# OAID/Tengine

Hardware: AMD Instinct MI355X
Metric: images/sec int8 MobileNet-v1 224x224 (higher is better)
Workload: dtype int8; 1 GPU; mobilenet_v1 int8 batch=1 per GPU (BASELINE configs[1]), weights = seeded synthetic tmfile, input resident in HBM, direct AQL dispatch of the launch list (14 packets per step), 1 stream(s); streams=1, halves=0, global_batch=1, parallelism=dp1, collectives=none

## Files before the change

include/tengine_amd.h:

```cpp
#ifndef TENGINE_AMD_H
#define TENGINE_AMD_H

#include <stddef.h>
#include <stdint.h>

#ifdef __cplusplus
extern "C" {
#endif

#define TAMD_API __attribute__((visibility("default")))

enum { TAMD_DT_FP32 = 0, TAMD_DT_FP16 = 1, TAMD_DT_INT8 = 2, TAMD_DT_UINT8 = 3, TAMD_DT_INT32 = 4 };
enum { TAMD_TT_VAR = 1, TAMD_TT_CONST = 2, TAMD_TT_INPUT = 3 };

enum {
    TAMD_OP_INPUT = 0,
    TAMD_OP_CONST = 1,
    TAMD_OP_CONV = 2,
    TAMD_OP_FC = 3,
    TAMD_OP_POOL = 4,
    TAMD_OP_RELU = 5,
    TAMD_OP_ELTWISE = 6,
    TAMD_OP_CONCAT = 7,
    TAMD_OP_DROPOUT = 8,
    TAMD_OP_UPSAMPLE = 9,
    TAMD_OP_RELU6 = 10,
    TAMD_OP_FLATTEN = 11,
    TAMD_OP_SOFTMAX = 12,
    TAMD_OP_PERMUTE = 13,
    TAMD_OP_RESHAPE = 14,
    TAMD_OP_PRIORBOX = 15,
    TAMD_OP_SIGMOID = 16,
    TAMD_OP_CLIP = 17,
    TAMD_OP_HARDSWISH = 18,
    TAMD_OP_MISH = 19,
    TAMD_OP_INTERP = 20,
    TAMD_OP_SPLIT = 22,
    TAMD_OP_SHUFFLECHANNEL = 23,
    TAMD_OP_PRELU = 25,
    TAMD_OP_SLICE = 26,
    TAMD_OP_NUM
};

typedef struct tamd_conv_param {
    int kernel_h, kernel_w, stride_h, stride_w;
    int pad_h0, pad_h1, pad_w0, pad_w1;
    int dilation_h, dilation_w;
    int input_channel, output_channel, group, activation;
} tamd_conv_param;

typedef struct tamd_fc_param { int num_output; } tamd_fc_param;

typedef struct tamd_pool_param {
    int pool_method, kernel_h, kernel_w, stride_h, stride_w;
    int pad_h0, pad_h1, pad_w0, pad_w1;
    int global, caffe_flavor;
} tamd_pool_param;

typedef struct tamd_relu_param { float negative_slope; } tamd_relu_param;
typedef struct tamd_eltwise_param { int type; int caffe_flavor; float shift, power, scale; } tamd_eltwise_param;
typedef struct tamd_concat_param { int axis; } tamd_concat_param;
typedef struct tamd_upsample_param { float scale; } tamd_upsample_param;
typedef struct tamd_permute_param { int order[4]; } tamd_permute_param;
typedef struct tamd_softmax_param { int axis; } tamd_softmax_param;
typedef struct tamd_reshape_param { int dim_num; int dims[8]; } tamd_reshape_param;
typedef struct tamd_clip_param { float max, min; } tamd_clip_param;
typedef struct tamd_hardswish_param { float alpha, beta; } tamd_hardswish_param;
typedef struct tamd_interp_param { int resize_type; float width_scale, height_scale; int output_width, output_height; } tamd_interp_param;
#define TAMD_SPLIT_MAX 8
typedef struct tamd_split_param { int axis; int num; int sizes[TAMD_SPLIT_MAX]; } tamd_split_param;
typedef struct tamd_shufflechannel_param { int group; } tamd_shufflechannel_param;
typedef struct tamd_slice_param {
    int axis, begin, end, step;
    int iscaffe, ismxnet, isonnx;
    int slice_point_num, begin_num, size_num;
} tamd_slice_param;

#define TAMD_PRIORBOX_MAX 8
typedef struct tamd_priorbox_param {
    int min_size_num, max_size_num, aspect_ratio_num;
    float min_size[TAMD_PRIORBOX_MAX], max_size[TAMD_PRIORBOX_MAX], aspect_ratio[TAMD_PRIORBOX_MAX], variance[4];
    int flip, clip, image_h, image_w;
    float step_h, step_w, offset;
} tamd_priorbox_param;

typedef struct tamd_tensor_desc {
    int dtype;
    int ttype;
    int dim_num;
    int dims[8];
    const void* data;
    int quant_num;
    const float* scales;
    const int* zero_points;
    const char* name;
} tamd_tensor_desc;

typedef struct tamd_node_desc {
    int op;
    int input_num;
    const int* inputs;
    int output_num;
    const int* outputs;
    const void* param;
    const char* name;
} tamd_node_desc;

typedef struct tamd_options {
    const char* dev_name;
    int size;
    int gpu_index;
    int use_hip_graph;
    int profile;
    int direct_dispatch;
    int keep_tensors;
    int u8_integer;
    int split_batch;
} tamd_options;
#define TAMD_OPTIONS_HAS(size, field) ((size) >= (int)(offsetof(tamd_options, field) + sizeof(((const tamd_options*)0)->field)))

typedef struct tamd_graph tamd_graph;

TAMD_API int tamd_device_count(void);
TAMD_API int tamd_init(int gpu_index);
TAMD_API int tamd_shutdown(void);
TAMD_API const char* tamd_last_error(void);
TAMD_API const char* tamd_version(void);
TAMD_API int tamd_op_supported(int op, int dtype);
TAMD_API int tamd_node_supported(const tamd_node_desc* node, const tamd_tensor_desc* inputs, int input_num,
                                 const tamd_tensor_desc* outputs, int output_num);
TAMD_API int tamd_lut_table(int op, int dtype, const void* param, float in_scale, int in_zp, float out_scale, int out_zp,
                            unsigned char table[256]);
TAMD_API int tamd_interp_table(int dtype, float in_scale, int in_zp, float out_scale, int out_zp, unsigned char table[256]);
TAMD_API int tamd_interp_indices(int in_extent, int out_extent, float scale, int* idx);
TAMD_API int tamd_shuffle_sources(int channels, int group, int* src);
TAMD_API int tamd_split_table(float in_scale, int in_zp, float out_scale, int out_zp, unsigned char table[256]);
TAMD_API int tamd_slice_table(float in_scale, int in_zp, float out_scale, int out_zp, unsigned char table[256]);
TAMD_API float tamd_prelu_slope(unsigned short half_bits);
TAMD_API int tamd_prelu_table(int dtype, unsigned short slope_bits, float in_scale, int in_zp, float out_scale, int out_zp,
                              unsigned char table[256]);

TAMD_API tamd_graph* tamd_graph_create(void);
TAMD_API int tamd_graph_add_tensor(tamd_graph* g, const tamd_tensor_desc* desc);
TAMD_API int tamd_graph_add_node(tamd_graph* g, const tamd_node_desc* desc);
TAMD_API int tamd_graph_set_inputs(tamd_graph* g, int n, const int* tensor_ids);
TAMD_API int tamd_graph_set_outputs(tamd_graph* g, int n, const int* tensor_ids);
TAMD_API tamd_graph* tamd_graph_load_tm2(const void* mem, size_t size);
TAMD_API int tamd_graph_set_batch(tamd_graph* g, int batch);

TAMD_API int tamd_graph_prerun(tamd_graph* g, const tamd_options* opt);
TAMD_API int tamd_graph_halves(const tamd_graph* g);
TAMD_API int tamd_graph_slots(const tamd_graph* g);
TAMD_API int tamd_graph_input_num(const tamd_graph* g);
TAMD_API int tamd_graph_output_num(const tamd_graph* g);
TAMD_API int tamd_graph_input_desc(const tamd_graph* g, int idx, int* dims8, int* dtype);
TAMD_API int tamd_graph_output_desc(const tamd_graph* g, int idx, int* dims8, int* dtype, float* scale, int* zero_point);
TAMD_API int tamd_graph_set_input(tamd_graph* g, int idx, const void* host_nchw, size_t bytes);
TAMD_API int tamd_graph_set_output(tamd_graph* g, int idx, void* host_nchw, size_t bytes);
TAMD_API int tamd_graph_run(tamd_graph* g);
TAMD_API int tamd_graph_run_async(tamd_graph* g);
TAMD_API int tamd_graph_wait(tamd_graph* g);
TAMD_API int tamd_graph_inflight(const tamd_graph* g);
TAMD_API int tamd_graph_upload_inputs(tamd_graph* g);
TAMD_API int tamd_graph_launch(tamd_graph* g);
TAMD_API int tamd_graph_sync(tamd_graph* g);
TAMD_API int tamd_graph_direct_packets(const tamd_graph* g);
TAMD_API int tamd_graph_direct_meta_packets(const tamd_graph* g);
TAMD_API int tamd_graph_direct_timestamps(tamd_graph* g, int passes, double* dur_us, double* gap_us, int max_packets);
TAMD_API const char* tamd_graph_direct_packet_name(const tamd_graph* g, int i);
TAMD_API int tamd_graph_slot_timestamps(tamd_graph* g, int passes, double* start_us, double* end_us, int max_stamps);
TAMD_API int tamd_graph_download_outputs(tamd_graph* g);
TAMD_API int tamd_graph_output_device(tamd_graph* g, int idx, void** dptr, size_t* bytes);
TAMD_API void* tamd_graph_stream(tamd_graph* g);
TAMD_API double tamd_graph_prerun_ms(const tamd_graph* g);
TAMD_API int tamd_graph_time_launches(tamd_graph* g, int iters, float* total_ms);

typedef struct tamd_kernel_info {
    char node[64];
    char kernel[48];
    double macs;
    double bytes;
    float ms;
} tamd_kernel_info;
TAMD_API int tamd_graph_kernel_num(const tamd_graph* g);
TAMD_API int tamd_graph_profile(tamd_graph* g, int iters, tamd_kernel_info* out, int max_out);
TAMD_API int tamd_graph_read_tensor(tamd_graph* g, int tensor_idx, void* host_nchw, size_t bytes);
TAMD_API int tamd_graph_tensor_num(const tamd_graph* g);
TAMD_API int tamd_graph_tensor_desc(const tamd_graph* g, int tensor_idx, int* dims8, int* dtype);

TAMD_API void tamd_graph_destroy(tamd_graph* g);

#ifdef __cplusplus
}
#endif
#endif
```

tengine_amd/capi.py:

```python
import ctypes as C
import os

import numpy as np

HERE = os.path.dirname(os.path.abspath(__file__))
LIB_PATH = os.path.join(HERE, "lib", "libtengine_amd.so")

DT_FP32, DT_FP16, DT_INT8, DT_UINT8, DT_INT32 = 0, 1, 2, 3, 4
_NP = {DT_FP32: np.float32, DT_FP16: np.float16, DT_INT8: np.int8, DT_UINT8: np.uint8, DT_INT32: np.int32}


class Options(C.Structure):
    _fields_ = [("dev_name", C.c_char_p), ("size", C.c_int), ("gpu_index", C.c_int), ("use_hip_graph", C.c_int), ("profile", C.c_int),
                ("direct_dispatch", C.c_int), ("keep_tensors", C.c_int), ("u8_integer", C.c_int), ("split_batch", C.c_int)]


class KernelInfo(C.Structure):
    _fields_ = [("node", C.c_char * 64), ("kernel", C.c_char * 48), ("macs", C.c_double), ("bytes", C.c_double),
                ("ms", C.c_float)]


EXPORTS = [
    "tamd_device_count", "tamd_init", "tamd_shutdown", "tamd_last_error", "tamd_version", "tamd_op_supported", "tamd_node_supported", "tamd_lut_table", "tamd_interp_table", "tamd_interp_indices", "tamd_shuffle_sources", "tamd_split_table", "tamd_slice_table", "tamd_prelu_slope", "tamd_prelu_table",
    "tamd_graph_create", "tamd_graph_add_tensor", "tamd_graph_add_node", "tamd_graph_set_inputs",
    "tamd_graph_set_outputs", "tamd_graph_load_tm2", "tamd_graph_set_batch", "tamd_graph_prerun", "tamd_graph_halves", "tamd_graph_slots",
    "tamd_graph_input_num", "tamd_graph_output_num", "tamd_graph_input_desc", "tamd_graph_output_desc",
    "tamd_graph_set_input", "tamd_graph_set_output", "tamd_graph_run", "tamd_graph_run_async", "tamd_graph_wait", "tamd_graph_inflight", "tamd_graph_upload_inputs",
    "tamd_graph_launch", "tamd_graph_sync", "tamd_graph_direct_packets", "tamd_graph_direct_meta_packets", "tamd_graph_download_outputs", "tamd_graph_output_device",
    "tamd_graph_direct_timestamps", "tamd_graph_slot_timestamps", "tamd_graph_direct_packet_name", "tamd_graph_stream", "tamd_graph_time_launches", "tamd_graph_prerun_ms", "tamd_graph_kernel_num", "tamd_graph_profile",
    "tamd_graph_read_tensor", "tamd_graph_tensor_num", "tamd_graph_tensor_desc", "tamd_graph_destroy",
]

_lib = None


class TamdError(RuntimeError):
    pass


def version():
    return lib().tamd_version().decode()


def lib():
    global _lib
    if _lib is None:
        if not os.path.exists(LIB_PATH):
            raise TamdError("native library %s is missing: run `python -c 'import __graft_entry__ as g; g.build()'` "
                            "(tengine_amd has no CPU fallback)" % LIB_PATH)
        L = C.CDLL(LIB_PATH)
        vp, ci = C.c_void_p, C.c_int
        L.tamd_last_error.restype = C.c_char_p
        L.tamd_version.restype = C.c_char_p
        L.tamd_graph_create.restype = vp
        L.tamd_graph_load_tm2.restype = vp
        L.tamd_graph_load_tm2.argtypes = [vp, C.c_size_t]
        L.tamd_graph_stream.restype = vp
        L.tamd_graph_direct_packet_name.restype = C.c_char_p
        L.tamd_graph_direct_packet_name.argtypes = [vp, ci]
        L.tamd_graph_direct_timestamps.argtypes = [vp, ci, C.POINTER(C.c_double), C.POINTER(C.c_double), ci]
        if hasattr(L, "tamd_graph_slots"):
            L.tamd_graph_slot_timestamps.argtypes = [vp, ci, C.POINTER(C.c_double), C.POINTER(C.c_double), ci]
            L.tamd_graph_slots.argtypes = [vp]
        L.tamd_graph_prerun_ms.restype = C.c_double
        L.tamd_graph_prerun_ms.argtypes = [vp]
        for name, args in {
            "tamd_graph_set_batch": [vp, ci], "tamd_graph_prerun": [vp, C.POINTER(Options)],
            "tamd_graph_input_num": [vp], "tamd_graph_output_num": [vp], "tamd_graph_halves": [vp],
            "tamd_graph_input_desc": [vp, ci, C.POINTER(ci), C.POINTER(ci)],
            "tamd_graph_output_desc": [vp, ci, C.POINTER(ci), C.POINTER(ci), C.POINTER(C.c_float), C.POINTER(ci)],
            "tamd_graph_set_input": [vp, ci, vp, C.c_size_t], "tamd_graph_set_output": [vp, ci, vp, C.c_size_t],
            "tamd_graph_run": [vp], "tamd_graph_run_async": [vp], "tamd_graph_wait": [vp], "tamd_graph_inflight": [vp],
            "tamd_graph_upload_inputs": [vp], "tamd_graph_launch": [vp],
            "tamd_graph_sync": [vp], "tamd_graph_direct_packets": [vp], "tamd_graph_direct_meta_packets": [vp], "tamd_graph_download_outputs": [vp],
            "tamd_graph_output_device": [vp, ci, C.POINTER(vp), C.POINTER(C.c_size_t)],
            "tamd_graph_stream": [vp], "tamd_graph_time_launches": [vp, ci, C.POINTER(C.c_float)],
            "tamd_graph_kernel_num": [vp], "tamd_graph_profile": [vp, ci, C.POINTER(KernelInfo), ci],
            "tamd_graph_read_tensor": [vp, ci, vp, C.c_size_t], "tamd_graph_tensor_num": [vp],
            "tamd_graph_tensor_desc": [vp, ci, C.POINTER(ci), C.POINTER(ci)], "tamd_graph_destroy": [vp],
            "tamd_init": [ci], "tamd_op_supported": [ci, ci],
        }.items():
            getattr(L, name).argtypes = args
        L.tamd_graph_destroy.restype = None
        L.tamd_lut_table.argtypes = [ci, ci, vp, C.c_float, ci, C.c_float, ci, C.POINTER(C.c_ubyte)]
        L.tamd_interp_table.argtypes = [ci, C.c_float, ci, C.c_float, ci, C.POINTER(C.c_ubyte)]
        L.tamd_interp_indices.argtypes = [ci, ci, C.c_float, C.POINTER(ci)]
        L.tamd_shuffle_sources.argtypes = [ci, ci, C.POINTER(ci)]
        L.tamd_split_table.argtypes = [C.c_float, ci, C.c_float, ci, C.POINTER(C.c_ubyte)]
        L.tamd_slice_table.argtypes = [C.c_float, ci, C.c_float, ci, C.POINTER(C.c_ubyte)]
        L.tamd_prelu_slope.argtypes = [C.c_ushort]
        L.tamd_prelu_slope.restype = C.c_float
        L.tamd_prelu_table.argtypes = [ci, C.c_ushort, C.c_float, ci, C.c_float, ci, C.POINTER(C.c_ubyte)]
        _lib = L
    return _lib


OP_SIGMOID, OP_CLIP, OP_HARDSWISH, OP_MISH = 16, 17, 18, 19
OP_INTERP = 20
OP_SPLIT, OP_SHUFFLECHANNEL = 22, 23
OP_PRELU = 25
OP_SLICE = 26


class SliceParam(C.Structure):
    _fields_ = [(k, C.c_int) for k in ("axis", "begin", "end", "step", "iscaffe", "ismxnet", "isonnx", "slice_point_num", "begin_num", "size_num")]


def slice_table(in_scale, in_zp, out_scale, out_zp):
    tab = (C.c_ubyte * 256)()
    rc = lib().tamd_slice_table(in_scale, in_zp, out_scale, out_zp, tab)
    return None if rc != 0 else np.frombuffer(tab, dtype=np.uint8).copy()
SPLIT_MAX = 8


class SplitParam(C.Structure):
    _fields_ = [("axis", C.c_int), ("num", C.c_int), ("sizes", C.c_int * SPLIT_MAX)]


class ShuffleChannelParam(C.Structure):
    _fields_ = [("group", C.c_int)]


def shuffle_sources(channels, group):
    src = (C.c_int * max(channels, 1))()
    rc = lib().tamd_shuffle_sources(channels, group, src)
    return None if rc != 0 else np.array(src[:channels], dtype=np.int32)


def prelu_slope(half_bits):
    return float(lib().tamd_prelu_slope(int(half_bits) & 0xffff))


def prelu_table(dtype, slope_bits, in_scale, in_zp, out_scale, out_zp):
    tab = (C.c_ubyte * 256)()
    rc = lib().tamd_prelu_table(dtype, int(slope_bits) & 0xffff, in_scale, in_zp, out_scale, out_zp, tab)
    return None if rc != 0 else np.frombuffer(tab, dtype=np.uint8).copy()


def split_table(in_scale, in_zp, out_scale, out_zp):
    tab = (C.c_ubyte * 256)()
    rc = lib().tamd_split_table(in_scale, in_zp, out_scale, out_zp, tab)
    return None if rc != 0 else np.frombuffer(tab, dtype=np.uint8).copy()


def interp_table(dtype, in_scale, in_zp, out_scale, out_zp):
    tab = (C.c_ubyte * 256)()
    rc = lib().tamd_interp_table(dtype, in_scale, in_zp, out_scale, out_zp, tab)
    return None if rc != 0 else np.frombuffer(tab, dtype=np.uint8).copy()


def interp_indices(in_extent, out_extent, scale):
    idx = (C.c_int * max(out_extent, 1))()
    rc = lib().tamd_interp_indices(in_extent, out_extent, scale, idx)
    return None if rc != 0 else np.array(idx[:out_extent], dtype=np.int32)


def lut_table(op, dtype, in_scale, in_zp, out_scale, out_zp, params=None):
    tab = (C.c_ubyte * 256)()
    p = (C.c_float * 2)(*params) if params is not None else None
    rc = lib().tamd_lut_table(op, dtype, C.cast(p, C.c_void_p) if p is not None else None, in_scale, in_zp, out_scale, out_zp, tab)
    return None if rc != 0 else np.frombuffer(tab, dtype=np.uint8).copy()


def _check(rc, what):
    if rc is None or (isinstance(rc, int) and rc < 0):
        raise TamdError("%s failed: %s" % (what, lib().tamd_last_error().decode()))
    return rc


def device_count():
    return lib().tamd_device_count()


class Graph:

    def __init__(self, tm_bytes: bytes, batch=None, gpu_index=0, use_hip_graph=True, profile=False, direct_dispatch=False, keep_tensors=False, u8_integer=False, split_batch=0):
        L = lib()
        self._h = L.tamd_graph_load_tm2(tm_bytes, len(tm_bytes))
        if not self._h:
            raise TamdError("tamd_graph_load_tm2 failed: %s" % L.tamd_last_error().decode())
        if batch is not None:
            _check(L.tamd_graph_set_batch(self._h, batch), "set_batch")
        opt = Options(b"HIP", C.sizeof(Options), gpu_index, 1 if use_hip_graph else 0, 1 if profile else 0, 1 if direct_dispatch else 0,
                      1 if keep_tensors else 0, 1 if u8_integer else 0, int(split_batch))
        _check(L.tamd_graph_prerun(self._h, C.byref(opt)), "prerun")
        self._in, self._out = [], []
        for i in range(L.tamd_graph_output_num(self._h)):
            dims = (C.c_int * 8)()
            dt, sc, zp = C.c_int(), C.c_float(), C.c_int()
            nd = L.tamd_graph_output_desc(self._h, i, dims, C.byref(dt), C.byref(sc), C.byref(zp))
            arr = np.zeros([dims[k] for k in range(nd)], _NP[dt.value])
            self._out.append(arr)
            _check(L.tamd_graph_set_output(self._h, i, arr.ctypes.data, arr.nbytes), "set_output")

    def halves(self):
        return lib().tamd_graph_halves(self._h)

    def slots(self):
        return lib().tamd_graph_slots(self._h) if hasattr(lib(), "tamd_graph_slots") else 0

    def slot_timestamps(self, passes=50):
        n = lib().tamd_graph_direct_packets(self._h)
        t0, t1 = (C.c_double * (passes * 2 * n))(), (C.c_double * (passes * 2 * n))()
        r = _check(lib().tamd_graph_slot_timestamps(self._h, passes, t0, t1, passes * 2 * n), "slot_timestamps")
        return (np.array(t0[:r * 2 * n]).reshape(r, 2, n), np.array(t1[:r * 2 * n]).reshape(r, 2, n))

    def input_desc(self, idx=0):
        dims = (C.c_int * 8)()
        dt = C.c_int()
        nd = lib().tamd_graph_input_desc(self._h, idx, dims, C.byref(dt))
        return [dims[k] for k in range(nd)], dt.value

    def set_input(self, arr, idx=0):
        arr = np.ascontiguousarray(arr)
        while len(self._in) <= idx:
            self._in.append(None)
        self._in[idx] = arr
        _check(lib().tamd_graph_set_input(self._h, idx, arr.ctypes.data, arr.nbytes), "set_input")

    def run(self):
        _check(lib().tamd_graph_run(self._h), "run")
        return [o.copy() for o in self._out]

    def run_noreturn(self):
        _check(lib().tamd_graph_run(self._h), "run")

    def run_async(self, out_arrays=None):
        if out_arrays is not None:
            for i, a in enumerate(out_arrays):
                _check(lib().tamd_graph_set_output(self._h, i, a.ctypes.data, a.nbytes), "set_output")
        _check(lib().tamd_graph_run_async(self._h), "run_async")

    def wait(self):
        _check(lib().tamd_graph_wait(self._h), "wait")

    def bind_default_outputs(self):
        for i, a in enumerate(self._out):
            _check(lib().tamd_graph_set_output(self._h, i, a.ctypes.data, a.nbytes), "set_output")

    def output_like(self):
        return [np.zeros_like(o) for o in self._out]

    def output_num(self):
        return lib().tamd_graph_output_num(self._h)

    def upload(self):
        _check(lib().tamd_graph_upload_inputs(self._h), "upload_inputs")

    def launch(self):
        _check(lib().tamd_graph_launch(self._h), "launch")

    def sync(self):
        _check(lib().tamd_graph_sync(self._h), "sync")

    def download(self):
        _check(lib().tamd_graph_download_outputs(self._h), "download_outputs")
        return [o.copy() for o in self._out]

    def time_launches(self, iters):
        ms = C.c_float()
        _check(lib().tamd_graph_time_launches(self._h, iters, C.byref(ms)), "time_launches")
        return ms.value

    def output_device(self, idx=0):
        p, n = C.c_void_p(), C.c_size_t()
        _check(lib().tamd_graph_output_device(self._h, idx, C.byref(p), C.byref(n)), "output_device")
        return p.value, n.value

    def stream(self):
        return lib().tamd_graph_stream(self._h)

    def prerun_ms(self):
        return lib().tamd_graph_prerun_ms(self._h)

    def direct_packets(self):
        return lib().tamd_graph_direct_packets(self._h)

    def direct_timestamps(self, passes=200):
        n = lib().tamd_graph_direct_packets(self._h)
        dur, gap = (C.c_double * n)(), (C.c_double * n)()
        _check(lib().tamd_graph_direct_timestamps(self._h, passes, dur, gap, n), "direct_timestamps")
        return [(lib().tamd_graph_direct_packet_name(self._h, i).decode(), dur[i], gap[i]) for i in range(n)]

    def direct_meta_packets(self):
        return lib().tamd_graph_direct_meta_packets(self._h)

    def kernel_num(self):
        return lib().tamd_graph_kernel_num(self._h)

    def profile(self, iters=10):
        n = lib().tamd_graph_kernel_num(self._h)
        arr = (KernelInfo * n)()
        _check(lib().tamd_graph_profile(self._h, iters, arr, n), "profile")
        return [dict(node=k.node.decode(), kernel=k.kernel.decode(), macs=k.macs, bytes=k.bytes, ms=k.ms) for k in arr]

    def read_tensor(self, idx):
        dims = (C.c_int * 8)()
        dt = C.c_int()
        nd = _check(lib().tamd_graph_tensor_desc(self._h, idx, dims, C.byref(dt)), "tensor_desc")
        arr = np.zeros([dims[k] for k in range(nd)], _NP[dt.value])
        _check(lib().tamd_graph_read_tensor(self._h, idx, arr.ctypes.data, arr.nbytes), "read_tensor")
        return arr

    def close(self):
        if self._h:
            lib().tamd_graph_destroy(self._h)
            self._h = None

    def __del__(self):
        try:
            self.close()
        except Exception:
            pass
```

tengine_amd/csrc/direct.cc:

```cpp
#include <hip/hip_runtime.h>
#include "env.h"
#include <hsa/hsa.h>
#include <hsa/hsa_ext_amd.h>
#include <hsa/hsa_ven_amd_loader.h>
#include <cxxabi.h>

#include <atomic>
#include <chrono>
#include <cstdio>
#include <cstdlib>
#include <cstring>
#include <map>
#include <mutex>
#include <string>

#include "codeobj_meta.h"
#include "launch_rec.h"

namespace tamd {

thread_local std::vector<LaunchRec>* g_launch_rec = nullptr;
thread_local bool g_launch_coherent = false;
thread_local bool g_launch_beside = false;

namespace {

struct KernelSym { uint64_t object; uint32_t kernarg, group, priv; };

struct DeviceCtx {
    bool tried = false, ok = false;
    hsa_agent_t agent{}, cpu{};
    bool have_cpu = false;
    std::map<std::string, KernelSym> syms;
    std::map<std::string, HiddenLayout> layouts;
    std::map<uint64_t, bool> seen_objects;
};
std::mutex g_mu;
std::map<int, DeviceCtx> g_ctx;
hsa_ven_amd_loader_1_03_pfn_t g_loader{};
bool g_loader_ok = false;

struct AgentPick { int want_bus, want_dev, index, seen; hsa_agent_t by_bdf, by_index, cpu; bool have_bdf, have_index, have_cpu; };

hsa_status_t pick_agent(hsa_agent_t a, void* data)
{
    AgentPick* p = (AgentPick*)data;
    hsa_device_type_t t;
    if (hsa_agent_get_info(a, HSA_AGENT_INFO_DEVICE, &t) != HSA_STATUS_SUCCESS) return HSA_STATUS_SUCCESS;
    if (t == HSA_DEVICE_TYPE_CPU && !p->have_cpu) { p->cpu = a; p->have_cpu = true; }
    if (t != HSA_DEVICE_TYPE_GPU) return HSA_STATUS_SUCCESS;
    uint32_t bdf = 0;
    if (hsa_agent_get_info(a, (hsa_agent_info_t)HSA_AMD_AGENT_INFO_BDFID, &bdf) == HSA_STATUS_SUCCESS
        && (int)((bdf >> 8) & 0xff) == p->want_bus && (int)((bdf >> 3) & 0x1f) == p->want_dev && !p->have_bdf) { p->by_bdf = a; p->have_bdf = true; }
    if (p->seen == p->index) { p->by_index = a; p->have_index = true; }
    p->seen++;
    return HSA_STATUS_SUCCESS;
}

struct SymScan { DeviceCtx* ctx; };

hsa_status_t scan_symbol(hsa_executable_t, hsa_agent_t, hsa_executable_symbol_t s, void* data)
{
    DeviceCtx* ctx = ((SymScan*)data)->ctx;
    hsa_symbol_kind_t kind;
    if (hsa_executable_symbol_get_info(s, HSA_EXECUTABLE_SYMBOL_INFO_TYPE, &kind) != HSA_STATUS_SUCCESS || kind != HSA_SYMBOL_KIND_KERNEL) return HSA_STATUS_SUCCESS;
    uint32_t len = 0;
    if (hsa_executable_symbol_get_info(s, HSA_EXECUTABLE_SYMBOL_INFO_NAME_LENGTH, &len) != HSA_STATUS_SUCCESS || len == 0 || len > 4096) return HSA_STATUS_SUCCESS;
    std::string name(len, '\0');
    if (hsa_executable_symbol_get_info(s, HSA_EXECUTABLE_SYMBOL_INFO_NAME, &name[0]) != HSA_STATUS_SUCCESS) return HSA_STATUS_SUCCESS;
    KernelSym k{};
    if (hsa_executable_symbol_get_info(s, HSA_EXECUTABLE_SYMBOL_INFO_KERNEL_OBJECT, &k.object) != HSA_STATUS_SUCCESS) return HSA_STATUS_SUCCESS;
    (void)hsa_executable_symbol_get_info(s, HSA_EXECUTABLE_SYMBOL_INFO_KERNEL_KERNARG_SEGMENT_SIZE, &k.kernarg);
    (void)hsa_executable_symbol_get_info(s, HSA_EXECUTABLE_SYMBOL_INFO_KERNEL_GROUP_SEGMENT_SIZE, &k.group);
    (void)hsa_executable_symbol_get_info(s, HSA_EXECUTABLE_SYMBOL_INFO_KERNEL_PRIVATE_SEGMENT_SIZE, &k.priv);
    ctx->syms[name] = k;
    return HSA_STATUS_SUCCESS;
}

hsa_status_t scan_code_object(hsa_executable_t, hsa_loaded_code_object_t lco, void* data)
{
    DeviceCtx* ctx = ((SymScan*)data)->ctx;
    if (!g_loader.hsa_ven_amd_loader_loaded_code_object_get_info) return HSA_STATUS_SUCCESS;
    uint32_t st = 0;
    if (g_loader.hsa_ven_amd_loader_loaded_code_object_get_info(lco, HSA_VEN_AMD_LOADER_LOADED_CODE_OBJECT_INFO_CODE_OBJECT_STORAGE_TYPE, &st) != HSA_STATUS_SUCCESS
        || st != HSA_VEN_AMD_LOADER_CODE_OBJECT_STORAGE_TYPE_MEMORY) return HSA_STATUS_SUCCESS;
    uint64_t base = 0, size = 0;
    if (g_loader.hsa_ven_amd_loader_loaded_code_object_get_info(lco, HSA_VEN_AMD_LOADER_LOADED_CODE_OBJECT_INFO_CODE_OBJECT_STORAGE_MEMORY_BASE, &base) != HSA_STATUS_SUCCESS
        || g_loader.hsa_ven_amd_loader_loaded_code_object_get_info(lco, HSA_VEN_AMD_LOADER_LOADED_CODE_OBJECT_INFO_CODE_OBJECT_STORAGE_MEMORY_SIZE, &size) != HSA_STATUS_SUCCESS
        || !base || !size) return HSA_STATUS_SUCCESS;
    if (ctx->seen_objects.count(base)) return HSA_STATUS_SUCCESS;
    ctx->seen_objects[base] = true;
    (void)codeobj_hidden_layouts((const void*)(uintptr_t)base, (size_t)size, ctx->layouts);
    return HSA_STATUS_SUCCESS;
}

hsa_status_t scan_executable(hsa_executable_t exe, void* data)
{
    DeviceCtx* ctx = ((SymScan*)data)->ctx;
    (void)hsa_executable_iterate_agent_symbols(exe, ctx->agent, scan_symbol, data);
    if (g_loader.hsa_ven_amd_loader_executable_iterate_loaded_code_objects)
        (void)g_loader.hsa_ven_amd_loader_executable_iterate_loaded_code_objects(exe, scan_code_object, data);
    return HSA_STATUS_SUCCESS;
}

void rescan(DeviceCtx* ctx)
{
    if (!g_loader_ok) return;
    SymScan sc{ctx};
    (void)g_loader.hsa_ven_amd_loader_iterate_executables(scan_executable, &sc);
}

DeviceCtx* device_ctx(int gpu)
{
    DeviceCtx& c = g_ctx[gpu];
    if (c.tried) return c.ok ? &c : nullptr;
    c.tried = true;
    if (hsa_init() != HSA_STATUS_SUCCESS) return nullptr;
    if (!g_loader_ok)
        g_loader_ok = hsa_system_get_major_extension_table(HSA_EXTENSION_AMD_LOADER, 1, sizeof(g_loader), &g_loader) == HSA_STATUS_SUCCESS
                      && g_loader.hsa_ven_amd_loader_iterate_executables != nullptr;
    if (!g_loader_ok) return nullptr;
    hipDeviceProp_t prop;
    if (hipGetDeviceProperties(&prop, gpu) != hipSuccess) return nullptr;
    AgentPick p{};
    p.want_bus = prop.pciBusID; p.want_dev = prop.pciDeviceID; p.index = gpu;
    if (hsa_iterate_agents(pick_agent, &p) != HSA_STATUS_SUCCESS) return nullptr;
    if (!p.have_bdf && !p.have_index) return nullptr;
    c.agent = p.have_bdf ? p.by_bdf : p.by_index;
    c.cpu = p.cpu; c.have_cpu = p.have_cpu;
    c.ok = true;
    return &c;
}

}

struct DirectQueue {
    hsa_queue_t* q = nullptr;
    hsa_signal_t done{};
    uint64_t bursts = 0;
    bool open = false;
    int refs = 0;
    std::atomic<int> fault{0};
    static constexpr hsa_signal_value_t kStart = (hsa_signal_value_t)1 << 40;
};

namespace {
thread_local char g_direct_err[256] = "";
void direct_err(const char* what, int code) { snprintf(g_direct_err, sizeof(g_direct_err), "%s (%d)", what, code); }

void queue_fault(hsa_status_t status, hsa_queue_t*, void* data)
{
    ((DirectQueue*)data)->fault.store((int)status ? (int)status : -1);
}

double wait_limit_s()
{
    static const double lim = getenv("TAMD_DIRECT_TIMEOUT_S") ? atof(getenv("TAMD_DIRECT_TIMEOUT_S")) : 30.0;
    return lim;
}
}

const char* direct_last_error() { return g_direct_err; }

bool direct_probe(int gpu)
{
    std::lock_guard<std::mutex> lk(g_mu);
    return device_ctx(gpu) != nullptr;
}

struct DirectProgram {
    DirectQueue* dq = nullptr;

    std::vector<hsa_kernel_dispatch_packet_t> pkts;
    std::vector<uint16_t> hdr;
    void* kernargs = nullptr;
    uint16_t h_open = 0, h_close = 0, h_wrap = 0;
    int n_meta = 0;
    hsa_agent_t agent{};
    std::vector<std::string> names;
};

DirectProgram* direct_build(int gpu, hipStream_t stream, const std::vector<LaunchRec>& recs, const char** why, DirectProgram* share)
{
    static const char* reason = "";
    *why = reason;
    if (recs.empty()) { *why = "empty launch list"; return nullptr; }
    std::lock_guard<std::mutex> lk(g_mu);
    DeviceCtx* ctx = device_ctx(gpu);
    if (!ctx) { *why = "no HSA agent / loader extension for this device"; return nullptr; }
    DirectProgram* p = new DirectProgram;
    std::vector<unsigned char> blob;
    std::vector<size_t> offs;
    std::vector<char> coherent;
    bool scanned = false;
    int n_meta = 0;
    for (const LaunchRec& r : recs) {
        const char* nm = hipKernelNameRefByPtr(r.func, stream);
        if (!nm) { *why = "kernel without a name"; delete p; return nullptr; }
        const std::string key = std::string(nm) + ".kd";
        auto it = ctx->syms.find(key);
        if (it == ctx->syms.end() && !scanned) { rescan(ctx); scanned = true; it = ctx->syms.find(key); }
        if (it == ctx->syms.end()) { *why = "kernel descriptor not found among the loaded code objects"; delete p; return nullptr; }
        const KernelSym& k = it->second;
        static const bool allow_scratch = !(exp_env("TAMD_DIRECT_SCRATCH") && atoi(exp_env("TAMD_DIRECT_SCRATCH")) == 0);
        if (k.priv != 0 && !allow_scratch) { *why = "a kernel of the list uses scratch memory"; delete p; return nullptr; }
        if (r.args.size() > k.kernarg) { *why = "recorded arguments exceed the kernel's argument segment"; delete p; return nullptr; }
        HiddenLayout hl;
        {
            static const bool use_meta = !(exp_env("TAMD_DIRECT_META") && atoi(exp_env("TAMD_DIRECT_META")) == 0);
            auto lt = ctx->layouts.find(key);
            if (use_meta && lt != ctx->layouts.end()) {
                hl = lt->second;
                if ((size_t)hl.explicit_end > ((r.args.size() + 7) & ~(size_t)7) || (size_t)hl.explicit_end + 8 < r.args.size()) {
                    *why = "recorded arguments do not match the kernel's metadata"; delete p; return nullptr;
                }
                n_meta++;
            } else {
                const int hid = (int)((r.args.size() + 7) & ~(size_t)7);
                for (int a3 = 0; a3 < 3; a3++) { hl.block_count[a3] = hid + 4 * a3; hl.group_size[a3] = hid + 12 + 2 * a3; hl.remainder[a3] = hid + 18 + 2 * a3; }
                hl.grid_dims = hid + 64;
            }
        }
        size_t seg = k.kernarg;
        for (int a3 = 0; a3 < 3; a3++) seg = std::max<size_t>(seg, std::max(hl.block_count[a3] + 4, std::max(hl.group_size[a3], hl.remainder[a3]) + 2));
        seg = std::max<size_t>(seg, std::max<size_t>(hl.grid_dims + 2, r.args.size()));
        const size_t off = (blob.size() + 255) & ~(size_t)255;
        blob.resize(off + seg, 0);
        memcpy(blob.data() + off, r.args.data(), r.args.size());
        const uint32_t bc[3] = {r.grid.x, r.grid.y, r.grid.z};
        const uint16_t gs[3] = {(uint16_t)r.block.x, (uint16_t)r.block.y, (uint16_t)r.block.z};
        const uint16_t dims = r.grid.z * r.block.z > 1 ? 3 : (r.grid.y * r.block.y > 1 ? 2 : 1), zero16 = 0;
        for (int a3 = 0; a3 < 3; a3++) {
            if (hl.block_count[a3] >= 0) memcpy(blob.data() + off + hl.block_count[a3], &bc[a3], 4);
            if (hl.group_size[a3] >= 0) memcpy(blob.data() + off + hl.group_size[a3], &gs[a3], 2);
            if (hl.remainder[a3] >= 0) memcpy(blob.data() + off + hl.remainder[a3], &zero16, 2);
        }
        if (hl.grid_dims >= 0) memcpy(blob.data() + off + hl.grid_dims, &dims, 2);
        offs.push_back(off);
        hsa_kernel_dispatch_packet_t pk{};
        pk.setup = (uint16_t)(dims << HSA_KERNEL_DISPATCH_PACKET_SETUP_DIMENSIONS);
        pk.workgroup_size_x = gs[0]; pk.workgroup_size_y = gs[1]; pk.workgroup_size_z = gs[2];
        pk.grid_size_x = r.grid.x * r.block.x; pk.grid_size_y = r.grid.y * r.block.y; pk.grid_size_z = r.grid.z * r.block.z;
        pk.private_segment_size = k.priv;
        pk.group_segment_size = k.group + r.shmem;
        pk.kernel_object = k.object;
        p->pkts.push_back(pk);
        {
            int st = 0;
            char* dm = abi::__cxa_demangle(nm, nullptr, nullptr, &st);
            p->names.push_back(st == 0 && dm ? std::string(dm) : std::string(nm));
            free(dm);
        }
        const bool allow_none = tamd_pin_int("direct_coherent", 1) != 0;
        coherent.push_back(allow_none && r.coherent);
    }
    if (hipMalloc(&p->kernargs, blob.size()) != hipSuccess || hipMemcpy(p->kernargs, blob.data(), blob.size(), hipMemcpyHostToDevice) != hipSuccess) {
        (void)hipGetLastError();
        *why = "kernel-argument buffer"; direct_destroy(p); return nullptr;
    }
    if (ctx->have_cpu) {
        hsa_agent_t both[2] = {ctx->agent, ctx->cpu};
        (void)hsa_amd_agents_allow_access(2, both, nullptr, p->kernargs);
    }
    for (size_t i = 0; i < p->pkts.size(); i++) p->pkts[i].kernarg_address = (char*)p->kernargs + offs[i];
    if (share) {
        p->dq = share->dq;
    } else {
        p->dq = new DirectQueue;
        uint32_t qsize = 1024;
        while (qsize < 8 * p->pkts.size()) qsize *= 2;
        if (hsa_queue_create(ctx->agent, qsize, HSA_QUEUE_TYPE_SINGLE, queue_fault, p->dq, UINT32_MAX, UINT32_MAX, &p->dq->q) != HSA_STATUS_SUCCESS) {
            *why = "hsa_queue_create"; p->dq->q = nullptr; p->dq->refs = 1; direct_destroy(p); return nullptr;
        }
        if (hsa_signal_create(DirectQueue::kStart, 0, nullptr, &p->dq->done) != HSA_STATUS_SUCCESS) { *why = "hsa_signal_create"; p->dq->refs = 1; direct_destroy(p); return nullptr; }
        if (const char* cm = exp_env("TAMD_DIRECT_CU_MASK")) {
            uint32_t mask[8] = {0, 0, 0, 0, 0, 0, 0, 0};
            if (!strcmp(cm, "first32")) mask[0] = 0xffffffffu;
            else if (!strcmp(cm, "stride8")) for (int i = 0; i < 8; i++) mask[i] = 0x01010101u;
            else if (!strcmp(cm, "first64")) mask[0] = mask[1] = 0xffffffffu;
            else if (!strcmp(cm, "stride4")) for (int i = 0; i < 8; i++) mask[i] = 0x11111111u;
            if (mask[0]) {
                const hsa_status_t st = hsa_amd_queue_cu_set_mask(p->dq->q, 256, mask);
                if (getenv("TAMD_DEBUG")) fprintf(stderr, "[tamd] direct queue CU mask %s: %s\n", cm, st == HSA_STATUS_SUCCESS ? "set" : "REFUSED");
            }
        }
    }
    p->dq->refs++;
    p->agent = ctx->agent;
    if (p->pkts.size() * 2 > p->dq->q->size) { *why = "launch list longer than the shared queue"; direct_destroy(p); return nullptr; }
    auto header = [](int type, int acq, int rel, bool barrier = true) {
        return (uint16_t)((type << HSA_PACKET_HEADER_TYPE) | ((barrier ? 1 : 0) << HSA_PACKET_HEADER_BARRIER) | (acq << HSA_PACKET_HEADER_SCACQUIRE_FENCE_SCOPE)
                          | (rel << HSA_PACKET_HEADER_SCRELEASE_FENCE_SCOPE));
    };
    const int K = HSA_PACKET_TYPE_KERNEL_DISPATCH;
    int n_beside = 0;
    for (size_t i = 0; i < p->pkts.size(); i++) {
        const bool beside = i > 0 && recs[i].beside;
        n_beside += beside;
        static const bool exp_nofence = exp_env("TAMD_EXP_NOFENCE") != nullptr;
        if (!coherent[i] && exp_nofence) p->hdr.push_back(header(K, HSA_FENCE_SCOPE_NONE, HSA_FENCE_SCOPE_NONE, !beside));
        else if (!coherent[i]) p->hdr.push_back(header(K, beside ? HSA_FENCE_SCOPE_NONE : HSA_FENCE_SCOPE_AGENT, HSA_FENCE_SCOPE_AGENT, !beside));
        else p->hdr.push_back(header(K, (i > 0 && !coherent[i - 1]) ? HSA_FENCE_SCOPE_AGENT : HSA_FENCE_SCOPE_NONE, HSA_FENCE_SCOPE_NONE));
    }
    if (getenv("TAMD_DEBUG")) fprintf(stderr, "[tamd] direct: %zu packets, %d without the barrier bit, hidden arguments of %d from code-object metadata\n", p->pkts.size(), n_beside, n_meta);
    p->n_meta = n_meta;
    p->h_open = header(K, HSA_FENCE_SCOPE_SYSTEM, coherent[0] ? HSA_FENCE_SCOPE_NONE : HSA_FENCE_SCOPE_AGENT);
    p->h_close = header(HSA_PACKET_TYPE_BARRIER_AND, HSA_FENCE_SCOPE_AGENT, HSA_FENCE_SCOPE_SYSTEM);
    p->h_wrap = (!recs.empty() && recs[0].wrap) ? (uint16_t)(p->hdr[0] & ~(1u << HSA_PACKET_HEADER_BARRIER)) : p->hdr[0];
    if (getenv("TAMD_DEBUG") && p->h_wrap != p->hdr[0]) fprintf(stderr, "[tamd] direct: the first launch of a pass runs beside the end of the previous pass\n");
    return p;
}

int direct_packets(const DirectProgram* p) { return p ? (int)p->pkts.size() : 0; }
const char* direct_packet_name(const DirectProgram* p, int i) { return (p && i >= 0 && i < (int)p->names.size()) ? p->names[i].c_str() : ""; }


static int submit_stamped(DirectProgram* p, const hsa_signal_t* sig)
{
    const int n = (int)p->pkts.size();
    DirectQueue* dq = p->dq;
    hsa_queue_t* q = dq->q;
    hsa_kernel_dispatch_packet_t* base = (hsa_kernel_dispatch_packet_t*)q->base_address;
    const uint64_t mask = q->size - 1;
    const uint64_t idx0 = hsa_queue_add_write_index_relaxed(q, (uint64_t)n);
    while (idx0 + n - hsa_queue_load_read_index_scacquire(q) > q->size)
        if (dq->fault.load()) return -1;
    for (int i = 0; i < n; i++) {
        hsa_kernel_dispatch_packet_t* d = base + ((idx0 + i) & mask);
        const hsa_kernel_dispatch_packet_t& s = p->pkts[i];
        d->setup = s.setup;
        d->workgroup_size_x = s.workgroup_size_x; d->workgroup_size_y = s.workgroup_size_y; d->workgroup_size_z = s.workgroup_size_z;
        d->reserved0 = 0;
        d->grid_size_x = s.grid_size_x; d->grid_size_y = s.grid_size_y; d->grid_size_z = s.grid_size_z;
        d->private_segment_size = s.private_segment_size; d->group_segment_size = s.group_segment_size;
        d->kernel_object = s.kernel_object; d->kernarg_address = s.kernarg_address; d->reserved2 = 0;
        d->completion_signal = sig[i];
        const uint16_t h = i == 0 ? (dq->open ? p->h_wrap : p->h_open) : p->hdr[i];
        __atomic_store_n(&d->header, h, __ATOMIC_RELEASE);
    }
    const uint64_t to_end = q->size - (idx0 & mask);
    if (to_end < (uint64_t)n) hsa_signal_store_screlease(q->doorbell_signal, (hsa_signal_value_t)(idx0 + to_end - 1));
    hsa_signal_store_screlease(q->doorbell_signal, (hsa_signal_value_t)(idx0 + n - 1));
    dq->open = true;
    return 0;
}

int direct_timestamps_two(DirectProgram* a, DirectProgram* b, int passes, double* start_us, double* end_us)
{
    const int n = (int)a->pkts.size();
    if (n == 0 || (int)b->pkts.size() != n || passes < 1 || a->dq == b->dq) { direct_err("two programs of the same list on two queues are needed", 0); return -1; }
    DirectProgram* prog[2] = {a, b};
    if (direct_wait_all(a) || direct_wait_all(b)) return -1;
    uint64_t freq = 0;
    if (hsa_system_get_info(HSA_SYSTEM_INFO_TIMESTAMP_FREQUENCY, &freq) != HSA_STATUS_SUCCESS || !freq) { direct_err("no timestamp frequency", 0); return -1; }
    for (DirectProgram* p : prog)
        if (hsa_amd_profiling_set_profiler_enabled(p->dq->q, 1) != HSA_STATUS_SUCCESS) { direct_err("hsa_amd_profiling_set_profiler_enabled", 0); return -1; }
    const int extra = 3, all = passes + extra;
    std::vector<hsa_signal_t> sig((size_t)all * 2 * n);
    for (auto& s : sig)
        if (hsa_signal_create(1, 0, nullptr, &s) != HSA_STATUS_SUCCESS) { direct_err("hsa_signal_create", 0); return -1; }
    int rc = 0;
    for (int ps = 0; ps < all && !rc; ps++) {
        for (int k = 0; k < 2 && !rc; k++) rc = submit_stamped(prog[k], &sig[((size_t)ps * 2 + k) * n]);
        if (ps + 1 == extra && !rc) rc = direct_wait(a) || direct_wait(b) ? -1 : 0;
    }
    if (!rc) rc = direct_wait(a) || direct_wait(b) ? -1 : 0;
    std::vector<uint64_t> t0(sig.size(), 0), t1(sig.size(), 0);
    for (size_t k = 0; k < sig.size() && !rc; k++) {
        hsa_amd_profiling_dispatch_time_t t{};
        if (hsa_amd_profiling_get_dispatch_time(a->agent, sig[k], &t) != HSA_STATUS_SUCCESS) { direct_err("hsa_amd_profiling_get_dispatch_time", (int)k); rc = -1; break; }
        t0[k] = t.start; t1[k] = t.end;
    }
    for (DirectProgram* p : prog) (void)hsa_amd_profiling_set_profiler_enabled(p->dq->q, 0);
    for (auto& s : sig) (void)hsa_signal_destroy(s);
    if (rc) return -1;
    int first_ok = extra;
    for (size_t k = 0; k < sig.size(); k++)
        if (t1[k] <= t0[k]) first_ok = std::max(first_ok, (int)(k / ((size_t)2 * n)) + 1);
    if (first_ok >= all) { direct_err("no round of the burst carries dispatch stamps throughout", all); return -1; }
    const size_t first = (size_t)first_ok * 2 * n;
    uint64_t origin = ~(uint64_t)0;
    for (size_t k = first; k < sig.size(); k++) origin = std::min(origin, t0[k]);
    for (size_t k = first; k < sig.size(); k++) {
        start_us[k - first] = 1e6 * (double)(t0[k] - origin) / (double)freq;
        end_us[k - first] = 1e6 * (double)(t1[k] - origin) / (double)freq;
    }
    return all - first_ok;
}

int direct_timestamps(DirectProgram* p, int passes, double* dur_us, double* gap_us)
{
    const int n = (int)p->pkts.size();
    if (n == 0 || passes < 1) return -1;
    DirectQueue* dq = p->dq;
    if (direct_wait_all(p)) return -1;
    uint64_t freq = 0;
    if (hsa_system_get_info(HSA_SYSTEM_INFO_TIMESTAMP_FREQUENCY, &freq) != HSA_STATUS_SUCCESS || !freq) { direct_err("no timestamp frequency", 0); return -1; }
    if (hsa_amd_profiling_set_profiler_enabled(dq->q, 1) != HSA_STATUS_SUCCESS) { direct_err("hsa_amd_profiling_set_profiler_enabled", 0); return -1; }
    passes += passes < 20 ? 3 : 1;
    std::vector<hsa_signal_t> sig((size_t)n * passes);
    for (auto& s : sig)
        if (hsa_signal_create(1, 0, nullptr, &s) != HSA_STATUS_SUCCESS) { direct_err("hsa_signal_create", 0); return -1; }
    int rc = 0;
    for (int ps = 0; ps < passes && !rc; ps++) {
        rc = submit_stamped(p, &sig[(size_t)ps * n]);
        if (ps == 0 && !rc) rc = direct_wait(p);
    }
    if (!rc) rc = direct_wait(p);
    std::vector<double> t0((size_t)n * passes, 0.0), t1((size_t)n * passes, 0.0);
    int first_ok = 1, n_bad = 0, last_bad = -1;
    for (size_t k = 0; k < sig.size() && !rc; k++) {
        hsa_amd_profiling_dispatch_time_t t{};
        if (hsa_amd_profiling_get_dispatch_time(p->agent, sig[k], &t) != HSA_STATUS_SUCCESS) { direct_err("hsa_amd_profiling_get_dispatch_time", (int)k); rc = -1; break; }
        if (getenv("TAMD_DEBUG") && k >= (size_t)n && k < (size_t)n + 4)
            fprintf(stderr, "[tamd] stamp %zu: start %llu end %llu (%lld ticks), system timestamp frequency %llu Hz\n", k, (unsigned long long)t.start,
                    (unsigned long long)t.end, (long long)(t.end - t.start), (unsigned long long)freq);
        if (t.end <= t.start) { first_ok = std::max(first_ok, (int)(k / (size_t)n) + 1); n_bad++; last_bad = (int)k; }
        const uint64_t origin = 0;
        t0[k] = 1e6 * (double)(t.start - origin) / (double)freq; t1[k] = 1e6 * (double)(t.end - origin) / (double)freq;
    }
    (void)hsa_amd_profiling_set_profiler_enabled(dq->q, 0);
    for (auto& s : sig) (void)hsa_signal_destroy(s);
    if (rc) return -1;
    if (first_ok >= passes) {
        char msg[200];
        snprintf(msg, sizeof(msg), "no pass carries dispatch stamps throughout: %d of %d packets without (the last one: packet %d of pass %d, %s)", n_bad, n * passes,
                 last_bad % n, last_bad / n, direct_packet_name(p, last_bad % n));
        direct_err(msg, passes - 1);
        return -1;
    }
    for (int i = 0; i < n; i++) {
        double d = 0, g = 0;
        int ng = 0;
        for (int ps = first_ok; ps < passes; ps++) {
            const size_t k = (size_t)ps * n + i;
            d += t1[k] - t0[k];
            if (k + 1 < sig.size()) { g += t0[k + 1] - t1[k]; ng++; }
        }
        dur_us[i] = d / (passes - first_ok);
        gap_us[i] = ng ? g / ng : 0.0;
    }
    return n;
}
int direct_meta_packets(const DirectProgram* p) { return p ? p->n_meta : 0; }

int direct_submit(DirectProgram* p, bool close_burst, unsigned long long* burst)
{
    const uint64_t n = p->pkts.size();
    DirectQueue* dq = p->dq;
    hsa_queue_t* q = dq->q;
    if (dq->fault.load()) { direct_err("the HSA queue is in the error state (a dispatched kernel faulted)", dq->fault.load()); return -1; }
    const uint64_t idx0 = hsa_queue_add_write_index_relaxed(q, n);
    if (idx0 + n - hsa_queue_load_read_index_scacquire(q) > q->size) {
        const auto t0 = std::chrono::steady_clock::now();
        while (idx0 + n - hsa_queue_load_read_index_scacquire(q) > q->size) {
            if (dq->fault.load() || std::chrono::duration<double>(std::chrono::steady_clock::now() - t0).count() > wait_limit_s()) {
                if (!dq->fault.load()) dq->fault.store(-2);
                direct_err("the HSA queue does not drain (faulted kernel or hung device)", dq->fault.load());
                return -1;
            }
        }
    }
    hsa_kernel_dispatch_packet_t* base = (hsa_kernel_dispatch_packet_t*)q->base_address;
    const uint64_t mask = q->size - 1;
    for (uint64_t i = 0; i < n; i++) {
        hsa_kernel_dispatch_packet_t* d = base + ((idx0 + i) & mask);
        const hsa_kernel_dispatch_packet_t& s = p->pkts[i];
        d->setup = s.setup;
        d->workgroup_size_x = s.workgroup_size_x; d->workgroup_size_y = s.workgroup_size_y; d->workgroup_size_z = s.workgroup_size_z;
        d->reserved0 = 0;
        d->grid_size_x = s.grid_size_x; d->grid_size_y = s.grid_size_y; d->grid_size_z = s.grid_size_z;
        d->private_segment_size = s.private_segment_size; d->group_segment_size = s.group_segment_size;
        d->kernel_object = s.kernel_object; d->kernarg_address = s.kernarg_address; d->reserved2 = 0;
        d->completion_signal.handle = 0;
        uint16_t h = i == 0 ? (dq->open ? p->h_wrap : p->h_open) : p->hdr[i];
        if (close_burst && i + 1 == n) {
            d->completion_signal = dq->done;
            h = (uint16_t)((h & ~(3u << HSA_PACKET_HEADER_SCRELEASE_FENCE_SCOPE)) | (HSA_FENCE_SCOPE_SYSTEM << HSA_PACKET_HEADER_SCRELEASE_FENCE_SCOPE)
                           | (1u << HSA_PACKET_HEADER_BARRIER));
        }
        __atomic_store_n(&d->header, h, __ATOMIC_RELEASE);
    }
    const uint64_t to_end = q->size - (idx0 & mask);
    if (to_end < n) hsa_signal_store_screlease(q->doorbell_signal, (hsa_signal_value_t)(idx0 + to_end - 1));
    hsa_signal_store_screlease(q->doorbell_signal, (hsa_signal_value_t)(idx0 + n - 1));
    if (close_burst) {
        dq->bursts++;
        dq->open = false;
        if (burst) *burst = dq->bursts;
    } else
        dq->open = true;
    return 0;
}

int direct_close(DirectProgram* p, unsigned long long* burst)
{
    DirectQueue* dq = p->dq;
    if (burst) *burst = dq->bursts;
    if (!dq->open) return 0;
    if (dq->fault.load()) { direct_err("the HSA queue is in the error state (a dispatched kernel faulted)", dq->fault.load()); return -1; }
    hsa_queue_t* q = dq->q;
    const uint64_t idx = hsa_queue_add_write_index_relaxed(q, 1);
    const auto t0 = std::chrono::steady_clock::now();
    while (idx + 1 - hsa_queue_load_read_index_scacquire(q) > q->size) {
        if (dq->fault.load() || std::chrono::duration<double>(std::chrono::steady_clock::now() - t0).count() > wait_limit_s()) {
            if (!dq->fault.load()) dq->fault.store(-2);
            direct_err("the HSA queue does not drain (faulted kernel or hung device)", dq->fault.load());
            return -1;
        }
    }
    hsa_barrier_and_packet_t* b = (hsa_barrier_and_packet_t*)q->base_address + (idx & (q->size - 1));
    b->reserved0 = 0; b->reserved1 = 0; b->reserved2 = 0;
    for (int i = 0; i < 5; i++) b->dep_signal[i].handle = 0;
    b->completion_signal = dq->done;
    __atomic_store_n(&b->header, p->h_close, __ATOMIC_RELEASE);
    hsa_signal_store_screlease(q->doorbell_signal, (hsa_signal_value_t)idx);
    dq->bursts++;
    dq->open = false;
    if (burst) *burst = dq->bursts;
    return 0;
}

int direct_wait_burst(DirectProgram* p, unsigned long long burst)
{
    DirectQueue* dq = p->dq;
    const hsa_signal_value_t target = DirectQueue::kStart - (hsa_signal_value_t)burst;
    if (hsa_signal_load_scacquire(dq->done) <= target) return 0;
    if (hsa_signal_wait_scacquire(dq->done, HSA_SIGNAL_CONDITION_LT, target + 1, 2000000 , HSA_WAIT_STATE_ACTIVE) <= target) return 0;
    const auto t0 = std::chrono::steady_clock::now();
    for (;;) {
        if (hsa_signal_wait_scacquire(dq->done, HSA_SIGNAL_CONDITION_LT, target + 1, 5000000, HSA_WAIT_STATE_BLOCKED) <= target) return 0;
        if (dq->fault.load()) { direct_err("a dispatched kernel faulted: the HSA queue is in the error state", dq->fault.load()); return -1; }
        if (std::chrono::duration<double>(std::chrono::steady_clock::now() - t0).count() > wait_limit_s()) {
            direct_err("timeout waiting for a direct pass (TAMD_DIRECT_TIMEOUT_S)", -3);
            return -1;
        }
    }
}

int direct_wait(DirectProgram* p)
{
    unsigned long long b = 0;
    if (!p->dq->open) return 0;
    if (direct_close(p, &b)) return -1;
    return direct_wait_burst(p, b);
}

int direct_wait_all(DirectProgram* p)
{
    if (direct_wait(p)) return -1;
    return direct_wait_burst(p, p->dq->bursts);
}

void direct_destroy(DirectProgram* p)
{
    if (!p) return;
    if (p->dq) {
        if (p->dq->q && !p->dq->fault.load()) (void)direct_wait_all(p);
        if (--p->dq->refs <= 0) {
            if (p->dq->q) (void)hsa_queue_destroy(p->dq->q);
            if (p->dq->done.handle) (void)hsa_signal_destroy(p->dq->done);
            delete p->dq;
        }
    }
    if (p->kernargs) (void)hipFree(p->kernargs);
    delete p;
}

}
```

tengine_amd/csrc/graph.h:

```cpp
#pragma once
#include <hip/hip_runtime.h>

#include <functional>
#include <atomic>
#include <map>
#include <string>
#include <vector>

#include "../../include/tengine_amd.h"
#include "graph_slots.h"
#include "kernels.h"
#include "node_rules.h"

namespace tamd {

void set_error(const char* fmt, ...);
static inline int rup(int v, int m) { return (v + m - 1) / m * m; }

struct HTensor {
    int dtype = 0, ttype = TAMD_TT_VAR;
    std::vector<int> dims;
    std::vector<uint8_t> data;
    std::vector<float> scales;
    std::vector<int> zps;
    std::string name;
    void* dptr = nullptr;
    int n = 0, h = 0, w = 0, c = 0;
    int cs = 0;
    int c_off = 0;
    bool is_view = false;
    bool nchw_raw = false;
    bool prerun_const = false;
    size_t elems() const { size_t e = 1; for (int d : dims) e *= (size_t)d; return e; }
};

union NodeParam {
    tamd_conv_param conv;
    tamd_fc_param fc;
    tamd_pool_param pool;
    tamd_relu_param relu;
    tamd_eltwise_param elt;
    tamd_concat_param concat;
    tamd_upsample_param ups;
    tamd_permute_param perm;
    tamd_softmax_param softmax;
    tamd_reshape_param reshape;
    tamd_priorbox_param priorbox;
    tamd_clip_param clip;
    tamd_hardswish_param hardswish;
    tamd_interp_param interp;
    tamd_split_param split;
    tamd_shufflechannel_param shuffle;
    tamd_slice_param slice;
};

struct HNode {
    int op = 0;
    std::vector<int> in, out;
    NodeParam p{};
    std::string name;
};

struct Access {
    const char* base = nullptr;
    size_t size = 0, off = 0, len = 0, period = 0;
};
inline bool access_overlap(const Access& a, const Access& b)
{
    if (a.base + a.size <= b.base || b.base + b.size <= a.base) return false;
    if (a.base == b.base && a.size == b.size && a.period > 0 && a.period == b.period) return !(a.off + a.len <= b.off || b.off + b.len <= a.off);
    return true;
}

struct Step {
    std::string node, kernel;
    double macs = 0, bytes = 0;
    std::function<hipError_t(hipStream_t)> fn;
    bool once = false;
    bool deps = false;
    std::vector<Access> rd, wr;
};
inline bool step_conflict(const Step& a, const Step& b)
{
    for (auto& w : a.wr) { for (auto& x : b.wr) if (access_overlap(w, x)) return true; for (auto& x : b.rd) if (access_overlap(w, x)) return true; }
    for (auto& r : a.rd) for (auto& x : b.wr) if (access_overlap(r, x)) return true;
    return false;
}
inline bool step_states_nothing(const Step& s) { return s.rd.empty() || s.wr.empty(); }
inline bool step_writes_what_it_reads(const Step& s)
{
    for (auto& w : s.wr)
        for (auto& r : s.rd)
            if (access_overlap(w, r)) return true;
    return false;
}
inline Step make_step(const std::string& node, const std::string& kernel, double macs, double bytes, std::function<hipError_t(hipStream_t)> fn,
                      std::vector<Access> rd, std::vector<Access> wr, bool deps)
{
    Step st;
    st.node = node; st.kernel = kernel; st.macs = macs; st.bytes = bytes; st.fn = std::move(fn);
    st.rd = std::move(rd); st.wr = std::move(wr); st.deps = deps;
    return st;
}
inline Access access_of(const HTensor& t)
{
    Access a;
    a.base = (const char*)t.dptr;
    const size_t esz = t.dtype == TAMD_DT_FP32 ? 4 : 1;
    if (t.nchw_raw || t.cs <= 0) {
        if (t.is_view && t.cs > 0) {
            a.period = (size_t)t.cs * t.h * t.w * esz; a.off = (size_t)t.c_off * t.h * t.w * esz; a.len = (size_t)t.c * t.h * t.w * esz;
            a.size = a.period * (size_t)t.n;
        } else {
            a.size = t.elems() * esz; a.len = a.size;
        }
    } else {
        a.size = (size_t)t.n * t.h * t.w * t.cs;
        if (t.is_view) { a.period = (size_t)t.cs; a.off = (size_t)t.c_off; a.len = (size_t)t.c; }
        else a.len = a.size;
    }
    return a;
}
inline Access access_of_bytes(const void* p, size_t bytes)
{
    Access a;
    a.base = (const char*)p; a.size = bytes; a.len = bytes;
    return a;
}

inline Access access_of_channels(const HTensor& t, int first, int count)
{
    Access a;
    a.base = (const char*)t.dptr;
    a.size = (size_t)t.n * t.h * t.w * t.cs;
    a.period = (size_t)t.cs; a.off = (size_t)(t.c_off + first); a.len = (size_t)count;
    return a;
}
inline Access access_of_slot(const HTensor& y, size_t period, size_t off, size_t len, size_t esz)
{
    Access a;
    a.base = (const char*)y.dptr;
    a.size = y.elems() * esz; a.period = period * esz; a.off = off * esz; a.len = len * esz;
    return a;
}

struct IOBind {
    int tensor = -1;
    const void* host_in = nullptr;
    void* host_out = nullptr;
    size_t bytes = 0;
    void* stage = nullptr;
    void* pinned[2] = {nullptr, nullptr};
};

struct IoSlot {
    DirectProgram* direct = nullptr;
    bool zero_copy = false;
    hipGraph_t hgraph = nullptr;
    hipGraphExec_t hexec[2] = {nullptr, nullptr};
    int next_exec = 0;
    hipEvent_t done = nullptr;
};

struct Inflight {
    int io_slot = 0;
    std::vector<void*> host_out;
    hipEvent_t done = nullptr;
    bool direct = false;
    unsigned long long burst = 0;
};

struct PoolGeom { int oh, ow, kh, kw, sh, sw, ph0, pw0; };

struct DevArena { char* base = nullptr; size_t cap = 0, used = 0; };

}

#define HIPCHK(expr)                                                                              \
    do {                                                                                          \
        hipError_t e_ = (expr);                                                                   \
        if (e_ != hipSuccess) {                                                                   \
            tamd::set_error("%s failed: %s (%s:%d)", #expr, hipGetErrorString(e_), __FILE__, __LINE__); \
            return -1;                                                                            \
        }                                                                                         \
    } while (0)

struct tamd_graph {
    std::atomic<unsigned long> owner{0};
    std::vector<tamd::HTensor> tensors;
    std::vector<tamd::HNode> nodes;
    std::vector<tamd::IOBind> inputs, outputs;
    std::vector<tamd::Step> steps;
    std::vector<tamd::Step> in_steps;
    std::vector<tamd::Step> out_steps;
    std::vector<void*> dev_allocs;
    std::vector<tamd::DevArena> arenas;
    std::vector<char> pooled;
    size_t pool_bytes = 0, unpooled_bytes = 0;
    std::map<int, float*> f32_copy;
    std::vector<char> fused_away;
    void* zero_page = nullptr;
    hipStream_t stream = nullptr;
    hipGraph_t hgraph = nullptr;
    hipGraphExec_t hexec = nullptr;
    hipGraphExec_t hexecs[4] = {nullptr, nullptr, nullptr, nullptr};
    int nexec = 0, next_exec = 0;
    tamd::IoSlot io[2];
    int next_io_slot = 0;
    std::vector<tamd::Inflight> inflight;
    tamd::DirectProgram* direct = nullptr;
    tamd::DirectProgram* direct1 = nullptr;
    void* slot_block = nullptr;
    std::vector<tamd::SlotSpan> slot_spans;
    int slot_turn = 0;
    bool slot_hold = false;
    bool had_once = false;
    int autotune_cold = -1;
    double prerun_ms = 0;
    bool direct_busy = false;
    bool stream_dirty = true;
    bool stream_exposed = false;
    int out_fresh_in = -1;
    long long h2h_ns[5] = {0, 0, 0, 0, 0};
    long long h2h_runs = 0;
    tamd_options opt{};
    bool prepared = false;
    int gpu = 0;
    tamd_graph* half[2] = {nullptr, nullptr};
    bool is_half = false;
    int formula_batch = 0;
    std::vector<void*> pair_out;
};

namespace tamd {

PoolGeom pool_geom(const tamd_pool_param& p, int h, int w);
int dev_alloc(tamd_graph* g, void** p, size_t bytes, bool zero);
struct RaceCand {
    std::string tag;
    std::function<hipError_t(hipStream_t)> fn;
    std::string name;
    std::function<bool()> live;
};
int plan_race(tamd_graph* g, const std::string& node, const std::vector<RaceCand>& cands, const std::string& key, float margin, bool tune);
int plan_cached(const std::string& key, const std::vector<RaceCand>& cands);
bool autotune_enabled();
void nhwc_geom(HTensor& t);
int append_steps(tamd_graph* g, const std::vector<Step>& launches);
int count_consumers(const tamd_graph* g, int tensor);
int plan_nchw_buffers(tamd_graph* g, size_t esz, const std::function<bool(const HNode& producer, const HTensor& x, const HTensor& cat)>& in_place);
int plan_nchw_outputs(tamd_graph* g, size_t esz);
int plan_lut(tamd_graph* g, HNode& n, std::vector<Step>* out);
int plan_interp(tamd_graph* g, HNode& n, std::vector<Step>* out);
int plan_split_u8(tamd_graph* g, HNode& n, std::vector<Step>* out);
int plan_shuffle_u8(tamd_graph* g, HNode& n, std::vector<Step>* out);
int plan_prelu(tamd_graph* g, HNode& n, std::vector<Step>* out);
const char* prelu_refusal_of(const tamd_graph* g, const HNode& n);
const char* slice_refusal_of(const tamd_graph* g, const HNode& n, bool check_out, SliceGeom* geom, unsigned char* table);
int slice_chain_next(const tamd_graph* g, size_t ni);
int plan_slice_u8(tamd_graph* g, HNode& n, int next, std::vector<Step>* out);
const char* eltwise_refusal_of(const tamd_graph* g, const HNode& n, int* gated);
int gate_lut_producer(const tamd_graph* g, const HNode& e, int gated);
int plan_chan_gate(tamd_graph* g, HNode& n, int gated, int lut_node, std::vector<Step>* out);
inline int nchw_out_img(const HTensor& t) { return (t.is_view ? t.cs : t.c) * t.h * t.w; }
struct AxisSplit { int axis = 0, outer = 1, on = 0, inner = 1; };
int axis_split(const std::vector<int>& dims, int axis, const char* what, const std::string& node, AxisSplit* s);
std::vector<unsigned> conv_tap_table(int K, int Kpad, int H, int W, int KH, int KW, int DH, int DW);
int priorbox_count(const tamd_priorbox_param& p);
void priorbox_eval(const tamd_priorbox_param& p, int feat_h, int feat_w, int data_h, int data_w, std::vector<float>* out);
void priorbox_quant_u8(const std::vector<float>& f, float scale, int zp, std::vector<uint8_t>* q);
void priorbox_quant_i8(const std::vector<float>& f, float scale, std::vector<int8_t>* q);
int plan_u8(tamd_graph* g);
int plan_f32(tamd_graph* g);

template <typename T>
int upload(tamd_graph* g, const std::vector<T>& host, T** dev)
{
    void* p = nullptr;
    if (dev_alloc(g, &p, host.size() * sizeof(T), false)) return -1;
    HIPCHK(hipMemcpyAsync(p, host.data(), host.size() * sizeof(T), hipMemcpyHostToDevice, g->stream));
    HIPCHK(hipStreamSynchronize(g->stream));
    *dev = (T*)p;
    return 0;
}

template <typename T>
int upload_bias(tamd_graph* g, const HTensor* b, int n, const T** dev)
{
    if (!b) return 0;
    std::vector<T> hb((const T*)b->data.data(), (const T*)b->data.data() + n);
    T* d = nullptr;
    if (upload(g, hb, &d)) return -1;
    *dev = d;
    return 0;
}

template <typename F>
int conv_f32_mfma_operands(tamd_graph* g, F32ConvArgs& a, int KH, int KW, int DH, int DW, F wk)
{
    a.cfg = conv_f32_mfma_pick(a);
    const int BM = conv_f32_mfma_bm(a.cfg), ntile = (a.cout + BM - 1) / BM, nstage = a.Kpad / 32, G = 64 / BM, NIg = 32 / G;
    std::vector<float> wf((size_t)ntile * nstage * 32 * BM, 0.f);
    for (int co = 0; co < a.cout; co++)
        for (int k = 0; k < a.K; k++) {
            const int r = k & 31;
            wf[(((size_t)(co / BM) * nstage + (k >> 5)) * NIg + r / G) * 64 + (r % G) * BM + co % BM] = wk(co, k);
        }
    float* dwf = nullptr; unsigned* dlut = nullptr;
    if (upload(g, wf, &dwf) || upload(g, conv_tap_table(a.K, a.Kpad, a.H, a.W, KH, KW, DH, DW), &dlut)) return -1;
    a.w = dwf; a.klut = dlut;
    return 0;
}

}
```

tengine_amd/csrc/graph.hip:

```cpp
#include "graph.h"
#include "graph_internal.h"
#include "env.h"

#include <stdarg.h>
#include <stddef.h>
#include <stdio.h>
#include <string.h>
#include <sys/stat.h>
#include <unistd.h>

#include <algorithm>
#include <cfloat>
#include <chrono>
#include <cmath>
#include <mutex>

#include "epilogue.h"

using namespace tamd;

static void dump_profile(tamd_graph* g)
{
    const int n = (int)g->steps.size();
    if (n == 0) return;
    std::vector<tamd_kernel_info> k(n);
    if (tamd_graph_profile(g, 10, k.data(), n) < 0) return;
    double tot = 0;
    for (auto& e : k) tot += e.ms;
    fprintf(stderr, "Tengine HIP device graph: %d launches, %.3f ms per run (sum of launches)\n", n, tot);
    for (int i = 0; i < n; i++)
        fprintf(stderr, "  %3d %-40s %-32s %8.2f us %6.2f%% %9.2f MMAC %9.1f KB\n", i, k[i].node, k[i].kernel, 1e3 * k[i].ms,
                tot > 0 ? 100.0 * k[i].ms / tot : 0.0, k[i].macs / 1e6, k[i].bytes / 1e3);
}

extern "C" {

int tamd_device_count(void)
{
    int n = 0;
    if (hipGetDeviceCount(&n) != hipSuccess) return 0;
    return n;
}

int tamd_init(int gpu_index)
{
    int n = tamd_device_count();
    if (n <= 0) { set_error("no HIP device visible: the tengine_amd backend needs an MI355X (it has no CPU fallback)"); return -1; }
    if (gpu_index < 0 || gpu_index >= n) { set_error("gpu_index %d out of range (%d devices)", gpu_index, n); return -1; }
    HIPCHK(hipSetDevice(gpu_index));
    return 0;
}

int tamd_shutdown(void) { return 0; }
const char* tamd_last_error(void) { return last_error(); }
const char* tamd_version(void) { return "tengine_amd 0.4 (gfx950)"; }

int tamd_op_supported(int op, int dtype)
{
    if (dtype != TAMD_DT_INT8 && dtype != TAMD_DT_UINT8 && dtype != TAMD_DT_FP32) return 0;
    if (op == TAMD_OP_UPSAMPLE) return 1;
    if (op == TAMD_OP_RELU6) return dtype == TAMD_DT_FP32;
    if (op == TAMD_OP_SOFTMAX) return 1;
    if (op == TAMD_OP_RESHAPE || op == TAMD_OP_PRIORBOX) return 1;
    if (op == TAMD_OP_PERMUTE) return dtype != TAMD_DT_FP32;
    if (is_lut_op(op)) return lut_op_on_device(op, dtype);
    if (op == TAMD_OP_INTERP) return interp_on_device(dtype);
    if (op == TAMD_OP_SPLIT || op == TAMD_OP_SHUFFLECHANNEL) return chanmap_on_device(dtype);
    if (op == TAMD_OP_SLICE) return slice_on_device(dtype);
    if (op == TAMD_OP_PRELU) return prelu_on_device(dtype);
    switch (op) {
    case TAMD_OP_INPUT: case TAMD_OP_CONST: case TAMD_OP_CONV: case TAMD_OP_FC: case TAMD_OP_POOL: case TAMD_OP_RELU:
    case TAMD_OP_ELTWISE: case TAMD_OP_CONCAT: case TAMD_OP_DROPOUT: case TAMD_OP_FLATTEN:
        return 1;
    default:
        return 0;
    }
}

int tamd_node_supported(const tamd_node_desc* n, const tamd_tensor_desc* in, int n_in, const tamd_tensor_desc* out, int n_out)
{
    if (!n || n_out < 1 || !out) return 0;
    const int dt = out[0].dtype;
    if (!tamd_op_supported(n->op, dt)) return 0;
    for (int i = 0; i < n_out; i++)
        if (out[i].dtype != dt || (dt != TAMD_DT_FP32 && out[i].quant_num != 1)) return 0;
    for (int i = 0; i < n_in; i++)
        if (in[i].ttype != TAMD_TT_CONST && (in[i].dtype != dt || (dt != TAMD_DT_FP32 && in[i].quant_num != 1))) return 0;
    auto elems = [](const tamd_tensor_desc& t) { size_t e = 1; for (int i = 0; i < t.dim_num; i++) e *= (size_t)t.dims[i]; return e; };
    switch (n->op) {
    case TAMD_OP_CONV: {
        if (n_in < 2 || !n->param || in[0].dim_num != 4 || in[1].dim_num != 4 || in[1].ttype != TAMD_TT_CONST) return 0;
        const tamd_conv_param& p = *(const tamd_conv_param*)n->param;
        const int cin = in[0].dims[1], cout = in[1].dims[0];
        const int kh = p.kernel_h ? p.kernel_h : 1, kw = p.kernel_w ? p.kernel_w : 1;
        if (p.group < 1 || cin % p.group || cout % p.group) return 0;
        if (elems(in[1]) != (size_t)cout * (cin / p.group) * kh * kw) return 0;
        if (in[1].quant_num != 0 && in[1].quant_num != 1 && in[1].quant_num != cout) return 0;
        if (dt != TAMD_DT_FP32 && in[1].quant_num == 0) return 0;
        if (dt == TAMD_DT_UINT8 && in[1].quant_num != 1) return 0;
        if (dt == TAMD_DT_INT8 && p.group == 1 && cin > 4 && !conv_i8_gemm_taps_fit(kh, kw)) return 0;
        if (n_in > 2 && (in[2].ttype != TAMD_TT_CONST || elems(in[2]) < (size_t)cout)) return 0;
        return 1;
    }
    case TAMD_OP_FC: {
        if (n_in < 2 || in[1].ttype != TAMD_TT_CONST || in[0].dim_num < 2) return 0;
        const size_t hidden = elems(in[0]) / (size_t)(in[0].dims[0] > 0 ? in[0].dims[0] : 1);
        const int nout = out[0].dim_num > 1 ? out[0].dims[1] : 0;
        if (nout < 1 || in[1].dim_num != 2 || in[1].dims[0] != nout || (size_t)in[1].dims[1] != hidden) return 0;
        if (n->param && ((const tamd_fc_param*)n->param)->num_output && ((const tamd_fc_param*)n->param)->num_output != nout) return 0;
        if (dt == TAMD_DT_UINT8 && !fc_u8_row_fits_lds(hidden)) return 0;
        return 1;
    }
    case TAMD_OP_ELTWISE: {
        if (n_in != 2 || !in) return 0;
        int gated = -1;
        if (eltwise_refusal((const tamd_eltwise_param*)n->param, dt, n_in, in[0].dim_num, in[0].dims, in[0].ttype == TAMD_TT_CONST, (size_t)in[0].quant_num, in[1].dim_num,
                            in[1].dims, in[1].ttype == TAMD_TT_CONST, (size_t)in[1].quant_num, (size_t)out[0].quant_num, &gated))
            return 0;
        const tamd_tensor_desc& big = in[gated == 1 ? 1 : 0];
        if (gated >= 0 && out[0].dim_num != big.dim_num) return 0;
        for (int i = 0; gated >= 0 && i < big.dim_num; i++) if (out[0].dims[i] != big.dims[i]) return 0;
        return 1;
    }
    case TAMD_OP_CONCAT: {
        int ax = n->param ? ((const tamd_concat_param*)n->param)->axis : 1;
        if (ax < 0) ax += out[0].dim_num;
        if (dt == TAMD_DT_INT8) {
            if (ax == 1) return out[0].dim_num >= 2;
            if (ax < 0 || ax >= out[0].dim_num) return 0;
            return out[0].dim_num != 4 || (out[0].dims[0] == 1 && out[0].dims[1] == 2 && out[0].dims[3] == 1);
        }
        return ax >= 0 && ax < out[0].dim_num;
    }
    case TAMD_OP_SOFTMAX: {
        if (dt != TAMD_DT_INT8) return 1;
        if (n_in < 1 || in[0].dim_num < 2 || in[0].dim_num > 4 || in[0].ttype == TAMD_TT_CONST) return 0;
        int ax = n->param ? ((const tamd_softmax_param*)n->param)->axis : 1;
        if (ax < 0) ax += in[0].dim_num;
        if (ax < 1 || ax >= in[0].dim_num) return 0;
        if (in[0].dim_num == 2 && ax != 1) return 0;
        return softmax_i8_axis_fits(in[0].dims[ax]);
    }
    case TAMD_OP_PRIORBOX: {
        if (!n->param || n_in < 2 || in[0].dim_num != 4 || in[1].dim_num != 4 || out[0].dim_num < 1 || out[0].dims[0] != 1) return 0;
        const tamd_priorbox_param& p = *(const tamd_priorbox_param*)n->param;
        return p.min_size_num >= 1 && p.min_size_num <= TAMD_PRIORBOX_MAX && p.aspect_ratio_num >= 0 && p.aspect_ratio_num <= TAMD_PRIORBOX_MAX
               && (p.max_size_num == 0 || p.max_size_num == p.min_size_num);
    }
    case TAMD_OP_PERMUTE: {
        if (!n->param || out[0].dim_num != 4) return 0;
        return permute_order_on_device(((const tamd_permute_param*)n->param)->order);
    }
    case TAMD_OP_UPSAMPLE: {
        const float sc = n->param ? ((const tamd_upsample_param*)n->param)->scale : 0.f;
        if (dt == TAMD_DT_INT8 && (n_in < 1 || in[0].dim_num != 4 || in[0].ttype == TAMD_TT_CONST)) return 0;
        return upsample_factor_on_device(sc);
    }
    case TAMD_OP_POOL: {
        if (!n->param || in[0].dim_num != 4) return 0;
        const int m = ((const tamd_pool_param*)n->param)->pool_method;
        return m == 0 || m == 1;
    }
    case TAMD_OP_SIGMOID: case TAMD_OP_CLIP: case TAMD_OP_HARDSWISH: case TAMD_OP_MISH: {
        if (n_in != 1 || in[0].ttype == TAMD_TT_CONST || in[0].dim_num < 1 || in[0].dim_num != out[0].dim_num) return 0;
        for (int i = 0; i < in[0].dim_num; i++) if (in[0].dims[i] != out[0].dims[i]) return 0;
        if (n->op == TAMD_OP_CLIP && !n->param) return 0;
        return lut_rank_on_device(n->op, in[0].dim_num);
    }
    case TAMD_OP_INTERP: {
        if (n_in < 1 || !in) return 0;
        InterpGeom geom;
        std::vector<int> iy, ix;
        if (interp_refusal((const tamd_interp_param*)n->param, dt, in[0].dim_num, in[0].dims, in[0].ttype == TAMD_TT_CONST, (size_t)in[0].quant_num,
                           (size_t)out[0].quant_num, &geom, &iy, &ix))
            return 0;
        return out[0].dim_num == 4 && out[0].dims[0] == in[0].dims[0] && out[0].dims[1] == in[0].dims[1] && out[0].dims[2] == geom.out_h
               && out[0].dims[3] == geom.out_w;
    }
    case TAMD_OP_SPLIT: {
        if (n_in < 1 || !in) return 0;
        const tamd_split_param* p = (const tamd_split_param*)n->param;
        std::vector<size_t> oq;
        for (int i = 0; i < n_out; i++) oq.push_back((size_t)out[i].quant_num);
        if (split_refusal(p, dt, in[0].dim_num, in[0].dims, in[0].ttype == TAMD_TT_CONST, (size_t)in[0].quant_num, n_out, oq.data())) return 0;
        for (int i = 0; i < n_out; i++)
            if (out[i].dim_num != 4 || out[i].dims[0] != in[0].dims[0] || out[i].dims[1] != p->sizes[i] || out[i].dims[2] != in[0].dims[2] || out[i].dims[3] != in[0].dims[3])
                return 0;
        return 1;
    }
    case TAMD_OP_SHUFFLECHANNEL: {
        if (n_in < 1 || !in) return 0;
        if (shuffle_refusal((const tamd_shufflechannel_param*)n->param, dt, in[0].dim_num, in[0].dims, in[0].ttype == TAMD_TT_CONST, (size_t)in[0].quant_num,
                            (size_t)out[0].quant_num))
            return 0;
        if (out[0].dim_num != 4) return 0;
        for (int i = 0; i < 4; i++) if (out[0].dims[i] != in[0].dims[i]) return 0;
        return 1;
    }
    case TAMD_OP_SLICE: {
        if (n_in < 1 || !in) return 0;
        return slice_refusal((const tamd_slice_param*)n->param, dt, in[0].dim_num, in[0].dims, in[0].ttype == TAMD_TT_CONST, (size_t)in[0].quant_num,
                             in[0].quant_num == 1 && in[0].scales ? in[0].scales[0] : 0.f, in[0].quant_num == 1 && in[0].zero_points ? in[0].zero_points[0] : 0, n_out,
                             (size_t)out[0].quant_num, out[0].quant_num == 1 && out[0].scales ? out[0].scales[0] : 0.f,
                             out[0].quant_num == 1 && out[0].zero_points ? out[0].zero_points[0] : 0, out[0].dim_num, out[0].dims, nullptr, nullptr)
               == nullptr;
    }
    case TAMD_OP_PRELU: {
        if (n_in < 2 || !in) return 0;
        if (prelu_refusal(dt, n_in, in[0].dim_num, in[0].dims, in[0].ttype == TAMD_TT_CONST, (size_t)in[0].quant_num, (size_t)out[0].quant_num, in[1].dtype,
                          in[1].ttype == TAMD_TT_CONST, elems(in[1]), in[1].data))
            return 0;
        if (out[0].dim_num != 4) return 0;
        for (int i = 0; i < 4; i++) if (out[0].dims[i] != in[0].dims[i]) return 0;
        return 1;
    }
    default:
        return 1;
    }
}

tamd_graph* tamd_graph_create(void) { return new tamd_graph(); }

int tamd_graph_add_tensor(tamd_graph* g, const tamd_tensor_desc* d)
{
    if (!g || !d) return -1;
    HTensor t;
    t.dtype = d->dtype; t.ttype = d->ttype;
    t.dims.assign(d->dims, d->dims + d->dim_num);
    if (d->name) t.name = d->name;
    if (d->quant_num > 0 && d->scales) {
        t.scales.assign(d->scales, d->scales + d->quant_num);
        if (d->zero_points) t.zps.assign(d->zero_points, d->zero_points + d->quant_num);
        else t.zps.assign(d->quant_num, 0);
    }
    if (d->ttype == TAMD_TT_CONST) {
        size_t bytes = t.elems() * esize(t.dtype);
        t.data.resize(bytes);
        if (d->data) memcpy(t.data.data(), d->data, bytes);
    }
    g->tensors.push_back(std::move(t));
    return (int)g->tensors.size() - 1;
}

int tamd_graph_add_node(tamd_graph* g, const tamd_node_desc* d)
{
    if (!g || !d) return -1;
    HNode n;
    n.op = d->op;
    if (d->op == TAMD_OP_SOFTMAX) n.p.softmax.axis = 1;
    if (d->name) n.name = d->name;
    for (int i = 0; i < d->input_num; i++) {
        if (d->inputs[i] < 0 || d->inputs[i] >= (int)g->tensors.size()) { set_error("node %s: bad input tensor", n.name.c_str()); return -1; }
        n.in.push_back(d->inputs[i]);
    }
    for (int i = 0; i < d->output_num; i++) {
        if (d->outputs[i] < 0 || d->outputs[i] >= (int)g->tensors.size()) { set_error("node %s: bad output tensor", n.name.c_str()); return -1; }
        n.out.push_back(d->outputs[i]);
    }
    if (d->param) {
        switch (d->op) {
        case TAMD_OP_CONV: n.p.conv = *(const tamd_conv_param*)d->param; break;
        case TAMD_OP_FC: n.p.fc = *(const tamd_fc_param*)d->param; break;
        case TAMD_OP_POOL: n.p.pool = *(const tamd_pool_param*)d->param; break;
        case TAMD_OP_RELU: n.p.relu = *(const tamd_relu_param*)d->param; break;
        case TAMD_OP_ELTWISE: n.p.elt = *(const tamd_eltwise_param*)d->param; break;
        case TAMD_OP_CONCAT: n.p.concat = *(const tamd_concat_param*)d->param; break;
        case TAMD_OP_UPSAMPLE: n.p.ups = *(const tamd_upsample_param*)d->param; break;
        case TAMD_OP_PERMUTE: n.p.perm = *(const tamd_permute_param*)d->param; break;
        case TAMD_OP_SOFTMAX: n.p.softmax = *(const tamd_softmax_param*)d->param; break;
        case TAMD_OP_RESHAPE: n.p.reshape = *(const tamd_reshape_param*)d->param; break;
        case TAMD_OP_PRIORBOX: n.p.priorbox = *(const tamd_priorbox_param*)d->param; break;
        case TAMD_OP_CLIP: n.p.clip = *(const tamd_clip_param*)d->param; break;
        case TAMD_OP_HARDSWISH: n.p.hardswish = *(const tamd_hardswish_param*)d->param; break;
        case TAMD_OP_INTERP: n.p.interp = *(const tamd_interp_param*)d->param; break;
        case TAMD_OP_SPLIT: n.p.split = *(const tamd_split_param*)d->param; break;
        case TAMD_OP_SHUFFLECHANNEL: n.p.shuffle = *(const tamd_shufflechannel_param*)d->param; break;
        case TAMD_OP_SLICE: n.p.slice = *(const tamd_slice_param*)d->param; break;
        default: break;
        }
    }
    g->nodes.push_back(std::move(n));
    return (int)g->nodes.size() - 1;
}

int tamd_graph_set_inputs(tamd_graph* g, int n, const int* ids)
{
    g->inputs.clear();
    for (int i = 0; i < n; i++) { IOBind b; b.tensor = ids[i]; g->inputs.push_back(b); }
    return 0;
}

int tamd_graph_set_outputs(tamd_graph* g, int n, const int* ids)
{
    g->outputs.clear();
    for (int i = 0; i < n; i++) { IOBind b; b.tensor = ids[i]; g->outputs.push_back(b); }
    return 0;
}

int tamd_graph_set_batch(tamd_graph* g, int batch)
{
    if (!g) { set_error("null graph"); return -1; }
    TAMD_ONE_THREAD(g);
    if (g->prepared) { set_error("set_batch after prerun"); return -1; }
    for (auto& io : g->inputs) g->tensors[io.tensor].dims[0] = batch;
    return 0;
}

static tamd_options resolve_options(const tamd_options* opt)
{
    tamd_options o{};
    o.dev_name = "HIP"; o.size = (int)sizeof(tamd_options); o.gpu_index = 0; o.use_hip_graph = 1; o.profile = 0;
    if (opt) {
        const int have = opt->size;
        if (TAMD_OPTIONS_HAS(have, gpu_index)) o.gpu_index = opt->gpu_index;
        if (TAMD_OPTIONS_HAS(have, use_hip_graph)) o.use_hip_graph = opt->use_hip_graph;
        if (TAMD_OPTIONS_HAS(have, profile)) o.profile = opt->profile;
        if (TAMD_OPTIONS_HAS(have, direct_dispatch)) o.direct_dispatch = opt->direct_dispatch;
        if (TAMD_OPTIONS_HAS(have, keep_tensors)) o.keep_tensors = opt->keep_tensors;
        if (TAMD_OPTIONS_HAS(have, u8_integer)) o.u8_integer = opt->u8_integer;
        if (TAMD_OPTIONS_HAS(have, split_batch)) o.split_batch = (opt->split_batch == 1 || opt->split_batch == 2) ? opt->split_batch : 0;
    }
    if (o.split_batch != 1)
        if (const char* sb = getenv("TAMD_SPLIT_BATCH")) { const int v = atoi(sb); o.split_batch = v == 0 ? 1 : v == 2 ? 2 : 0; }
    if (const char* ui = getenv("TAMD_U8_INT")) o.u8_integer = atoi(ui) != 0;
    if (const char* dd = getenv("TAMD_DIRECT_DISPATCH")) o.direct_dispatch = atoi(dd) != 0;
    if (o.direct_dispatch && !getenv("TAMD_DIRECT_UNDER_TOOLS")) {
        const char* pre = getenv("LD_PRELOAD");
        if (getenv("HSA_TOOLS_LIB") || getenv("ROCP_TOOL_LIBRARIES") || getenv("ROCPROFILER_LIBRARY") || (pre && strstr(pre, "rocprof"))) o.direct_dispatch = 0;
    }
    if (const char* dt = getenv("TG_DEBUG_TIME")) { if (atoi(dt) == 1) o.profile = 1; }
    return o;
}

static int capture_pass(tamd_graph* g, int io_slot, hipGraph_t* out)
{
    HIPCHK(hipStreamBeginCapture(g->stream, hipStreamCaptureModeThreadLocal));
    const int rc = run_steps(g, g->stream, io_slot);
    const hipError_t e = hipStreamEndCapture(g->stream, out);
    if (rc) return -1;
    HIPCHK(e);
    return 0;
}

static int capture_graphs(tamd_graph* g)
{
    if (run_steps(g, g->stream)) return -1;
    HIPCHK(hipStreamSynchronize(g->stream));
    if (capture_pass(g, -1, &g->hgraph)) return -1;
    const char* ne = exp_env("TAMD_GRAPH_EXECS");
    g->nexec = ne ? std::max(1, std::min(4, atoi(ne))) : 3;
    for (int i = 0; i < g->nexec; i++) HIPCHK(hipGraphInstantiate(&g->hexecs[i], g->hgraph, nullptr, nullptr, 0));
    g->hexec = g->hexecs[0];
    const char* ioenv = exp_env("TAMD_IO_GRAPH");
    for (int io_slot = 0; io_slot < 2 && !(ioenv && atoi(ioenv) == 0); io_slot++) {
        IoSlot& s = g->io[io_slot];
        if (capture_pass(g, io_slot, &s.hgraph)) return -1;
        for (auto& e : s.hexec) HIPCHK(hipGraphInstantiate(&e, s.hgraph, nullptr, nullptr, 0));
    }
    return 0;
}

static int build_direct_programs(tamd_graph* g)
{
    std::vector<LaunchRec> recs;
    if (record_pass(g, -1, &recs)) return -1;
    const char* why = "";
    g->direct = direct_build(g->gpu, g->stream, recs, &why);
    if (!g->direct) fprintf(stderr, "tengine_amd: direct dispatch not used (hipGraph replay instead): %s\n", why);
    if (g->direct && !exp_env("TAMD_EXP_NOFENCE") && direct_selfcheck(g)) {
        fprintf(stderr, "tengine_amd: direct dispatch DISABLED for this graph: %s (hipGraph replay instead)\n", last_error());
        direct_destroy(g->direct);
        g->direct = nullptr;
    }
    if (!g->direct) return 0;
    for (int io_slot = 0; io_slot < 2 && g->io[io_slot].hexec[0]; io_slot++)
        if (build_io_program(g, io_slot)) return -1;
    if (!g->io[0].direct && g->io[1].direct) { direct_destroy(g->io[1].direct); g->io[1].direct = nullptr; }
    if (g->opt.split_batch != 1) slots_try_build(g, recs, g->opt.split_batch);
    if (getenv("TAMD_DEBUG") && g->io[0].direct)
        fprintf(stderr, "[tamd] host-to-host list: %d packets%s\n", direct_packets(g->io[0].direct), g->io[0].zero_copy ? ", outputs stored straight into the pinned host buffers" : "");
    return 0;
}

int tamd_graph_prerun(tamd_graph* g, const tamd_options* opt)
{
    TAMD_ONE_THREAD(g);
    if (!g) return -1;
    if (g->prepared) return 0;
    if (const int pr = pair_try_prerun(g, opt)) return pr < 0 ? -1 : 0;
    std::lock_guard<std::mutex> lk(g_capture_mutex);
    tamd_options o = resolve_options(opt);
    const auto prerun_t0 = std::chrono::steady_clock::now();
    g->opt = o;
    if (infer_shapes(g) || validate_graph(g)) return -1;
    if (tamd_init(o.gpu_index)) return -1;
    if (o.direct_dispatch && !(o.use_hip_graph && direct_probe(o.gpu_index))) { o.direct_dispatch = 0; g->opt = o; }
    g->gpu = o.gpu_index;
    HIPCHK(hipStreamCreateWithFlags(&g->stream, hipStreamNonBlocking));
    bool any_u8 = false, any_f32 = false, any_i8 = false;
    for (auto& t : g->tensors)
        if (t.ttype != TAMD_TT_CONST) (t.dtype == TAMD_DT_UINT8 ? any_u8 : t.dtype == TAMD_DT_FP32 ? any_f32 : any_i8) = true;
    if ((int)any_u8 + (int)any_f32 + (int)any_i8 > 1) { set_error("mixed int8 / uint8 / fp32 activations in one device graph"); return -1; }
    if (any_u8 ? plan_u8(g) : any_f32 ? plan_f32(g) : plan_i8(g)) return -1;
    for (auto& st : g->steps)
        if (st.once) { HIPCHK(st.fn(g->stream)); g->had_once = true; }
    g->steps.erase(std::remove_if(g->steps.begin(), g->steps.end(), [](const Step& st) { return st.once; }), g->steps.end());
    for (auto* v : {&g->inputs, &g->outputs})
        for (auto& io : *v)
            for (int s = 0; s < 2; s++) HIPCHK(hipHostMalloc(&io.pinned[s], std::max<size_t>(io.bytes, 16), hipHostMallocDefault));
    HIPCHK(hipDeviceSynchronize());
    if (o.use_hip_graph && capture_graphs(g)) return -1;
    if (o.use_hip_graph && o.direct_dispatch && build_direct_programs(g)) return -1;
    plan_cache_flush();
    g->prerun_ms = std::chrono::duration<double, std::milli>(std::chrono::steady_clock::now() - prerun_t0).count();
    g->prepared = true;
    return 0;
}

int tamd_graph_halves(const tamd_graph* g) { return g && g->half[0] ? 2 : 0; }
int tamd_graph_slots(const tamd_graph* g) { return g && !g->half[0] && g->direct && g->direct1 ? 2 : 0; }
int tamd_graph_input_num(const tamd_graph* g) { return (int)g->inputs.size(); }
int tamd_graph_output_num(const tamd_graph* g) { return (int)g->outputs.size(); }

static int fill_desc(const HTensor& t, int* dims8, int* dtype)
{
    for (size_t i = 0; i < t.dims.size() && i < 8; i++) dims8[i] = t.dims[i];
    if (dtype) *dtype = t.dtype;
    return (int)t.dims.size();
}

int tamd_graph_input_desc(const tamd_graph* g, int idx, int* dims8, int* dtype)
{
    if (idx < 0 || idx >= (int)g->inputs.size()) return -1;
    return fill_desc(g->tensors[g->inputs[idx].tensor], dims8, dtype);
}

int tamd_graph_output_desc(const tamd_graph* g, int idx, int* dims8, int* dtype, float* scale, int* zp)
{
    if (idx < 0 || idx >= (int)g->outputs.size()) return -1;
    const HTensor& t = g->tensors[g->outputs[idx].tensor];
    if (scale) *scale = t.scales.empty() ? 0.f : t.scales[0];
    if (zp) *zp = t.zps.empty() ? 0 : t.zps[0];
    return fill_desc(t, dims8, dtype);
}

int tamd_graph_set_input(tamd_graph* g, int idx, const void* host, size_t bytes)
{
    if (!g) { set_error("null graph"); return -1; }
    TAMD_ONE_THREAD(g);
    if (idx < 0 || idx >= (int)g->inputs.size()) { set_error("bad input index"); return -1; }
    if (g->prepared && bytes != g->inputs[idx].bytes) { set_error("input %d: %zu bytes given, %zu expected", idx, bytes, g->inputs[idx].bytes); return -1; }
    if (g->half[0]) return pair_set_input(g, idx, host, bytes);
    g->inputs[idx].host_in = host;
    return 0;
}

int tamd_graph_set_output(tamd_graph* g, int idx, void* host, size_t bytes)
{
    if (!g) { set_error("null graph"); return -1; }
    TAMD_ONE_THREAD(g);
    if (idx < 0 || idx >= (int)g->outputs.size()) { set_error("bad output index"); return -1; }
    if (g->prepared && bytes != g->outputs[idx].bytes) { set_error("output %d: %zu bytes given, %zu expected", idx, bytes, g->outputs[idx].bytes); return -1; }
    if (g->half[0]) return pair_set_output(g, idx, host, bytes);
    g->outputs[idx].host_out = host;
    return 0;
}


int tamd_graph_kernel_num(const tamd_graph* g) { return g->half[0] ? pair_kernel_num(g) : (int)g->steps.size(); }

int tamd_graph_profile(tamd_graph* g, int iters, tamd_kernel_info* out, int max_out)
{
    TAMD_ONE_THREAD(g);
    if (bind_device(g)) return -1;
    if (!g->prepared) { set_error("graph not prepared"); return -1; }
    if (g->half[0]) return pair_profile(g, iters, out, max_out);
    if (!g->inflight.empty()) { set_error("tamd_graph_profile while asynchronous runs are in flight: collect them with tamd_graph_wait first"); return -1; }
    if (direct_drain(g)) return -1;
    g->out_fresh_in = -1;
    int n = std::min((int)g->steps.size(), max_out);
    std::vector<hipEvent_t> ev(2 * g->steps.size());
    for (auto& e : ev) HIPCHK(hipEventCreate(&e));
    std::vector<double> acc(g->steps.size(), 0.0);
    for (size_t i = 0; i < g->steps.size(); i++) {
        HIPCHK(hipEventRecord(ev[2 * i], g->stream));
        for (int it = 0; it < iters; it++) {
            hipError_t e = g->steps[i].fn(g->stream);
            if (e != hipSuccess) { set_error("profile launch failed: %s", hipGetErrorString(e)); return -1; }
        }
        HIPCHK(hipEventRecord(ev[2 * i + 1], g->stream));
    }
    HIPCHK(hipStreamSynchronize(g->stream));
    for (size_t i = 0; i < g->steps.size(); i++) {
        float ms = 0;
        HIPCHK(hipEventElapsedTime(&ms, ev[2 * i], ev[2 * i + 1]));
        acc[i] = (double)ms;
    }
    if (run_steps(g, g->stream)) return -1;
    HIPCHK(hipStreamSynchronize(g->stream));
    for (auto& e : ev) hipEventDestroy(e);
    for (int i = 0; i < n; i++) {
        memset(&out[i], 0, sizeof(out[i]));
        snprintf(out[i].node, sizeof(out[i].node), "%s", g->steps[i].node.c_str());
        snprintf(out[i].kernel, sizeof(out[i].kernel), "%s", g->steps[i].kernel.c_str());
        out[i].macs = g->steps[i].macs;
        out[i].bytes = g->steps[i].bytes;
        out[i].ms = (float)(acc[i] / iters);
    }
    return n;
}

int tamd_graph_tensor_num(const tamd_graph* g) { return (int)g->tensors.size(); }

int tamd_graph_tensor_desc(const tamd_graph* g, int idx, int* dims8, int* dtype)
{
    if (idx < 0 || idx >= (int)g->tensors.size()) return -1;
    return fill_desc(g->tensors[idx], dims8, dtype);
}

int tamd_graph_read_tensor(tamd_graph* g, int idx, void* host, size_t bytes)
{
    if (!g) { set_error("null graph"); return -1; }
    TAMD_ONE_THREAD(g);
    if (idx < 0 || idx >= (int)g->tensors.size() || !g->prepared) return -1;
    if (bind_device(g)) return -1;
    if (g->half[0]) return pair_read_tensor(g, idx, host, bytes);
    HTensor& t = g->tensors[idx];
    if (t.ttype == TAMD_TT_CONST) { memcpy(host, t.data.data(), std::min(bytes, t.data.size())); return 0; }
    if ((size_t)idx < g->fused_away.size() && g->fused_away[idx]) {
        set_error("read_tensor: %s was fused into its consumer's launch and never reaches memory (TAMD_FUSE_PWDW=0 / "
                  "TAMD_FUSE_ELTWISE=0 / TAMD_FUSE_RELU=0 at prerun materialise it)", t.name.c_str());
        return -1;
    }
    if ((size_t)idx < g->pooled.size() && g->pooled[idx]) {
        set_error("read_tensor: %s shares its device memory with tensors of other lifetimes and does not survive the pass "
                  "(tamd_options.keep_tensors = 1 / TAMD_POOL=0 at prerun gives every tensor its own buffer)", t.name.c_str());
        return -1;
    }
    size_t need = t.elems() * esize(t.dtype);
    if (bytes != need) { set_error("read_tensor: %zu bytes given, %zu needed", bytes, need); return -1; }
    if (g->out_fresh_in >= 0)
        for (auto& io : g->outputs)
            if (io.tensor == idx && io.stage == t.dptr && stage_from_pinned(g)) return -1;
    if (direct_drain(g)) return -1;
    HIPCHK(hipStreamSynchronize(g->stream));
    if (t.nchw_raw && t.is_view) {
        const size_t es = esize(t.dtype), img = (size_t)t.c * t.h * t.w * es;
        HIPCHK(hipMemcpy2DAsync(host, img, (const char*)t.dptr + (size_t)t.c_off * t.h * t.w * es, (size_t)t.cs * t.h * t.w * es, img,
                                (size_t)t.n, hipMemcpyDeviceToHost, g->stream));
        HIPCHK(hipStreamSynchronize(g->stream));
        return 0;
    }
    if (t.nchw_raw) {
        HIPCHK(hipMemcpyAsync(host, t.dptr, need, hipMemcpyDeviceToHost, g->stream));
        HIPCHK(hipStreamSynchronize(g->stream));
        return 0;
    }
    void* tmp = nullptr;
    HIPCHK(hipMalloc(&tmp, need));
    LayoutArgs a{(const int8_t*)t.dptr + t.c_off, tmp, t.n, t.c, t.h, t.w, t.cs, esize(t.dtype)};
    hipError_t e = launch_nhwc_to_nchw(a, g->stream);
    if (e != hipSuccess) { hipFree(tmp); set_error("layout launch failed"); return -1; }
    HIPCHK(hipMemcpyAsync(host, tmp, need, hipMemcpyDeviceToHost, g->stream));
    HIPCHK(hipStreamSynchronize(g->stream));
    { std::lock_guard<std::mutex> lk(g_capture_mutex); hipFree(tmp); }
    return 0;
}

void tamd_graph_destroy(tamd_graph* g)
{
    if (!g) return;
    if (g->half[0]) { pair_destroy(g); return; }
    if (g->prepared) (void)bind_device(g);
    if (g->prepared && g->opt.profile) dump_profile(g);
    if (g->h2h_runs > 0)
        fprintf(stderr, "[tamd] blocking run, host side, mean of %lld runs (us): copy in %.2f | stream drain %.2f | submit %.2f | wait %.2f | copy out %.2f\n", g->h2h_runs,
                1e-3 * g->h2h_ns[0] / g->h2h_runs, 1e-3 * g->h2h_ns[1] / g->h2h_runs, 1e-3 * g->h2h_ns[2] / g->h2h_runs, 1e-3 * g->h2h_ns[3] / g->h2h_runs,
                1e-3 * g->h2h_ns[4] / g->h2h_runs);
    g->inflight.clear();
    if (g->stream) hipStreamSynchronize(g->stream);
    std::lock_guard<std::mutex> lk(g_capture_mutex);
    direct_teardown(g);
    for (int i = 0; i < g->nexec; i++) if (g->hexecs[i]) hipGraphExecDestroy(g->hexecs[i]);
    for (auto& s : g->io) {
        for (auto& e : s.hexec) if (e) hipGraphExecDestroy(e);
        if (s.hgraph) hipGraphDestroy(s.hgraph);
    }
    if (g->hgraph) hipGraphDestroy(g->hgraph);
    for (void* p : g->dev_allocs) hipFree(p);
    for (auto* v : {&g->inputs, &g->outputs})
        for (auto& io : *v)
            for (void* p : io.pinned) if (p) hipHostFree(p);
    for (auto& s : g->io) if (s.done) hipEventDestroy(s.done);
    if (g->stream) hipStreamDestroy(g->stream);
    delete g;
}

}
```

tengine_amd/csrc/graph_exec.hip:

```cpp
#include "graph.h"
#include "graph_internal.h"
#include "env.h"

#include <stdio.h>
#include <string.h>

#include <algorithm>
#include <chrono>

namespace tamd {

int run_steps(tamd_graph* g, hipStream_t s, int io_slot)
{
    if (io_slot >= 0)
        for (auto& io : g->inputs) {
            hipError_t e = launch_copy_bytes(io.stage, io.pinned[io_slot], io.bytes, s);
            if (e != hipSuccess) { set_error("input upload launch failed: %s", hipGetErrorString(e)); return -1; }
        }
    const char* ov_env = exp_env("TAMD_DIRECT_OVERLAP");
    const bool overlap = g_launch_rec && ov_env && atoi(ov_env) == 1;
    const char* wr_env = exp_env("TAMD_DIRECT_WRAP");
    const bool wrap = g_launch_rec && io_slot < 0 && wr_env && atoi(wr_env) == 1;
    const size_t rec0 = g_launch_rec ? g_launch_rec->size() : 0;
    const Step *first_step = nullptr, *last_step = nullptr;
    size_t last_step_recs = 0;
    std::vector<const Step*> open;
    for (auto* v : {&g->in_steps, &g->steps, &g->out_steps})
        for (auto& st : *v) {
            if (overlap) {
                bool beside = st.deps && !open.empty();
                for (size_t i = 0; i < open.size() && beside; i++) beside = open[i]->deps && !step_conflict(st, *open[i]);
                if (beside) launch_rec_beside();
                else open.clear();
                open.push_back(&st);
            }
            const size_t before = g_launch_rec ? g_launch_rec->size() : 0;
            hipError_t e = st.fn(s);
            launch_rec_clear_flags();
            if (e != hipSuccess) { set_error("launch %s (%s) failed: %s", st.kernel.c_str(), st.node.c_str(), hipGetErrorString(e)); return -1; }
            if (!first_step) first_step = &st;
            last_step = &st;
            last_step_recs = g_launch_rec ? g_launch_rec->size() - before : 0;
        }
    if (wrap && first_step && last_step && first_step != last_step && first_step->deps && last_step->deps && last_step_recs == 1
        && !(overlap && open.size() > 1) && !step_conflict(*first_step, *last_step) && g_launch_rec->size() > rec0)
        (*g_launch_rec)[rec0].wrap = true;
    if (io_slot >= 0)
        for (auto& io : g->outputs) {
            hipError_t e = launch_copy_bytes(io.pinned[io_slot], io.stage, io.bytes, s);
            if (e != hipSuccess) { set_error("output download launch failed: %s", hipGetErrorString(e)); return -1; }
        }
    return 0;
}

static int launch_io(tamd_graph* g, int io_slot)
{
    IoSlot& s = g->io[io_slot];
    if (s.hexec[0]) {
        hipGraphExec_t e = s.hexec[s.next_exec];
        s.next_exec ^= 1;
        HIPCHK(hipGraphLaunch(e, g->stream));
        return 0;
    }
    return run_steps(g, g->stream, io_slot);
}

int record_pass(tamd_graph* g, int io_slot, std::vector<LaunchRec>* recs)
{
    recs->clear();
    g_launch_rec = recs;
    const int rc = run_steps(g, g->stream, io_slot);
    g_launch_rec = nullptr;
    if (rc) return -1;
    HIPCHK(hipStreamSynchronize(g->stream));
    return 0;
}

int selfcheck_fill_inputs(tamd_graph* g, unsigned seed, int io_slot)
{
    std::vector<unsigned char> noise;
    unsigned lcg = seed;
    for (auto& io : g->inputs) {
        noise.resize(io.bytes);
        if (g->tensors[io.tensor].dtype == TAMD_DT_FP32) {
            float* f = (float*)noise.data();
            for (size_t i = 0; i < io.bytes / 4; i++) { lcg = lcg * 1664525u + 1013904223u; f[i] = (float)((int)(lcg >> 20) - 2048) / 1024.f; }
        } else
            for (size_t i = 0; i < io.bytes; i++) { lcg = lcg * 1664525u + 1013904223u; noise[i] = (unsigned char)(lcg >> 24); }
        if (io_slot >= 0) memcpy(io.pinned[io_slot], noise.data(), io.bytes);
        else HIPCHK(hipMemcpy(io.stage, noise.data(), io.bytes, hipMemcpyHostToDevice));
    }
    return 0;
}

int selfcheck_snapshot(const tamd_graph* g, OutputBytes* dst, int io_slot, const std::vector<SlotSpan>* spans)
{
    dst->clear();
    for (auto& io : g->outputs) {
        dst->emplace_back(io.bytes);
        if (io_slot >= 0) { memcpy(dst->back().data(), io.pinned[io_slot], io.bytes); continue; }
        const void* src = spans ? (const void*)slot_moved(*spans, (uintptr_t)io.stage) : io.stage;
        HIPCHK(hipMemcpy(dst->back().data(), src, io.bytes, hipMemcpyDeviceToHost));
    }
    return 0;
}

int selfcheck_same(const OutputBytes& want, const OutputBytes& got, const char* fmt)
{
    for (size_t i = 0; i < want.size(); i++)
        if (want[i] != got[i]) { set_error(fmt, i); return -1; }
    return 0;
}

int direct_selfcheck(tamd_graph* g)
{
    OutputBytes want, got;
    if (selfcheck_fill_inputs(g, 0x5EED1234u) || run_steps(g, g->stream)) return -1;
    HIPCHK(hipStreamSynchronize(g->stream));
    if (selfcheck_snapshot(g, &want)) return -1;
    if (selfcheck_fill_inputs(g, 0x0BADF00Du) || run_steps(g, g->stream)) return -1;
    HIPCHK(hipStreamSynchronize(g->stream));
    if (selfcheck_fill_inputs(g, 0x5EED1234u)) return -1;
    HIPCHK(hipDeviceSynchronize());
    if (direct_submit(g->direct) || direct_wait(g->direct)) { set_error("direct pass failed: %s", direct_last_error()); return -1; }
    if (selfcheck_snapshot(g, &got)) return -1;
    for (auto& io : g->inputs) HIPCHK(hipMemset(io.stage, 0, io.bytes));
    HIPCHK(hipDeviceSynchronize());
    return selfcheck_same(want, got, "the direct pass does not reproduce the eager pass (output %zu differs)");
}

static int patch_pointer(std::vector<LaunchRec>& recs, size_t nrecs, const void* from, const void* to)
{
    int hits = 0;
    for (size_t r = 0; r < nrecs; r++)
        for (size_t off = 0; off + 8 <= recs[r].args.size(); off += 8) {
            const void* v;
            memcpy(&v, recs[r].args.data() + off, 8);
            if (v == from) { memcpy(recs[r].args.data() + off, &to, 8); hits++; }
        }
    return hits;
}

static bool zero_copy_outputs(tamd_graph* g, std::vector<LaunchRec>& recs, int io_slot)
{
    const char* e = getenv("TAMD_IO_ZERO_COPY");
    const size_t nout = g->outputs.size();
    if ((e && atoi(e) == 0) || nout == 0 || recs.size() <= nout + g->inputs.size()) return false;
    const size_t body = recs.size() - nout;
    std::vector<LaunchRec> trial(recs.begin(), recs.begin() + body);
    for (auto& io : g->outputs) {
        const HTensor& t = g->tensors[io.tensor];
        if (io.stage == t.dptr && count_consumers(g, io.tensor) != 1) return false;
        if (t.prerun_const) return false;
        void* dev = nullptr;
        if (hipHostGetDevicePointer(&dev, io.pinned[io_slot], 0) != hipSuccess) { (void)hipGetLastError(); return false; }
        if (patch_pointer(trial, body, io.stage, dev) < 1) return false;
    }
    recs.swap(trial);
    return true;
}

static bool zero_copy_inputs(tamd_graph* g, std::vector<LaunchRec>& recs, int io_slot)
{
    const char* e = exp_env("TAMD_IO_ZERO_COPY_IN");
    const size_t nin = g->inputs.size();
    if (!(e && atoi(e) == 1) || nin == 0 || recs.size() <= nin) return false;
    std::vector<LaunchRec> trial(recs.begin() + nin, recs.end());
    for (auto& io : g->inputs) {
        void* dev = nullptr;
        if (hipHostGetDevicePointer(&dev, io.pinned[io_slot], 0) != hipSuccess) { (void)hipGetLastError(); return false; }
        if (patch_pointer(trial, trial.size(), io.stage, dev) < 1) return false;
    }
    recs.swap(trial);
    return true;
}

static int direct_io_selfcheck(tamd_graph* g, DirectProgram* pio, int io_slot)
{
    OutputBytes want, got;
    if (selfcheck_fill_inputs(g, 0xC0FFEE11u + (unsigned)io_slot, io_slot) || run_steps(g, g->stream, io_slot)) return -1;
    HIPCHK(hipStreamSynchronize(g->stream));
    if (selfcheck_snapshot(g, &want, io_slot)) return -1;
    for (auto& io : g->outputs) memset(io.pinned[io_slot], 0xA5, io.bytes);
    HIPCHK(hipDeviceSynchronize());
    unsigned long long b = 0;
    if (direct_submit(pio, true, &b) || direct_wait_burst(pio, b)) { set_error("direct host-to-host pass failed: %s", direct_last_error()); return -1; }
    if (selfcheck_snapshot(g, &got, io_slot)) return -1;
    return selfcheck_same(want, got, "the direct host-to-host pass does not reproduce the eager list (output %zu differs)");
}

int build_io_program(tamd_graph* g, int io_slot)
{
    std::vector<LaunchRec> recs;
    if (record_pass(g, io_slot, &recs)) return -1;
    const std::vector<LaunchRec> with_downloads = recs;
    bool zc = zero_copy_outputs(g, recs, io_slot);
    if (zero_copy_inputs(g, recs, io_slot)) zc = true;
    const char* why = "";
    DirectProgram* pio = direct_build(g->gpu, g->stream, recs, &why, g->direct);
    if (pio && direct_io_selfcheck(g, pio, io_slot)) {
        if (zc) fprintf(stderr, "tengine_amd: zero-copy outputs DISABLED for this graph: %s\n", last_error());
        direct_destroy(pio);
        why = last_error();
        pio = zc ? direct_build(g->gpu, g->stream, with_downloads, &why, g->direct) : nullptr;
        zc = false;
        if (pio && direct_io_selfcheck(g, pio, io_slot)) { direct_destroy(pio); pio = nullptr; why = last_error(); }
    }
    if (!pio) fprintf(stderr, "tengine_amd: direct dispatch not used for host-to-host runs (slot %d): %s\n", io_slot, why);
    g->io[io_slot].direct = pio;
    g->io[io_slot].zero_copy = zc && pio;
    return 0;
}


int bind_device(tamd_graph* g)
{
    if (!g) { set_error("null graph"); return -1; }
    HIPCHK(hipSetDevice(g->gpu));
    return 0;
}

int direct_drain(tamd_graph* g)
{
    if (g->direct && g->direct_busy) {
        if (direct_wait(g->direct) || (g->direct1 && direct_wait(g->direct1))) { set_error("direct dispatch: %s", direct_last_error()); return -1; }
        g->direct_busy = false;
    }
    g->slot_turn = 0;
    return 0;
}

void direct_teardown(tamd_graph* g)
{
    for (int s = 1; s >= 0; s--)
        if (g->io[s].direct) { direct_destroy(g->io[s].direct); g->io[s].direct = nullptr; }
    slots_destroy(g);
    if (g->direct) { direct_destroy(g->direct); g->direct = nullptr; }
}

static int direct_abandon(tamd_graph* g)
{
    set_error("direct dispatch: %s", direct_last_error());
    fprintf(stderr, "tengine_amd: direct dispatch abandoned for this graph (%s): hipGraph replay from here on\n", last_error());
    g->inflight.erase(std::remove_if(g->inflight.begin(), g->inflight.end(), [](const Inflight& f) { return f.direct; }), g->inflight.end());
    direct_teardown(g);
    g->direct_busy = false;
    return -1;
}

static inline long long now_ns() { return std::chrono::duration_cast<std::chrono::nanoseconds>(std::chrono::steady_clock::now().time_since_epoch()).count(); }
static bool close_on_last_packet()
{
    const char* e = tamd_pin("direct_close_on_last");
    return !(e && atoi(e) == 0);
}

static int submit_burst(DirectProgram* p, unsigned long long* burst)
{
    return close_on_last_packet() ? direct_submit(p, true, burst) : (direct_submit(p) || direct_close(p, burst));
}

static int drain_stream_if_pending(tamd_graph* g)
{
    if (g->stream_dirty || g->stream_exposed) { HIPCHK(hipStreamSynchronize(g->stream)); g->stream_dirty = false; }
    return 0;
}

int stage_from_pinned(tamd_graph* g)
{
    if (g->out_fresh_in < 0) return 0;
    if (!g->inflight.empty()) { set_error("the outputs of the last host-to-host run live in a pinned buffer that a run in flight may overwrite: tamd_graph_wait first"); return -1; }
    if (direct_drain(g)) return -1;
    for (auto& io : g->outputs)
        HIPCHK(hipMemcpyAsync(io.stage, io.pinned[g->out_fresh_in], io.bytes, hipMemcpyHostToDevice, g->stream));
    HIPCHK(hipStreamSynchronize(g->stream));
    g->out_fresh_in = -1;
    return 0;
}

}

using namespace tamd;

extern "C" {

int tamd_graph_upload_inputs(tamd_graph* g)
{
    TAMD_ONE_THREAD(g);
    if (bind_device(g)) return -1;
    if (g->half[0]) return pair_both(g, tamd_graph_upload_inputs);
    if (!g->inflight.empty()) { set_error("tamd_graph_upload_inputs while asynchronous runs are in flight (they own the pinned buffers): collect them with tamd_graph_wait first"); return -1; }
    if (direct_drain(g)) return -1;
    if (!g->prepared) { set_error("graph not prepared"); return -1; }
    for (auto& io : g->inputs) {
        if (!io.host_in) { set_error("input buffer not set"); return -1; }
        memcpy(io.pinned[0], io.host_in, io.bytes);
        HIPCHK(hipMemcpyAsync(io.stage, io.pinned[0], io.bytes, hipMemcpyHostToDevice, g->stream));
    }
    g->stream_dirty = true;
    return 0;
}

int tamd_graph_launch(tamd_graph* g)
{
    TAMD_ONE_THREAD(g);
    if (bind_device(g)) return -1;
    if (!g->prepared) { set_error("graph not prepared"); return -1; }
    if (g->half[0]) return pair_both(g, tamd_graph_launch);
    g->out_fresh_in = -1;
    if (g->direct) {
        if (!g->direct_busy) { HIPCHK(hipStreamSynchronize(g->stream)); g->stream_dirty = false; }
        g->direct_busy = true;
        DirectProgram* p = g->direct;
        if (g->direct1 && !g->slot_hold) { if (g->slot_turn) p = g->direct1; g->slot_turn ^= 1; }
        if (direct_submit(p)) { set_error("direct dispatch: %s", direct_last_error()); return -1; }
        return 0;
    }
    g->stream_dirty = true;
    if (g->hexec) {
        hipGraphExec_t e = g->hexecs[g->next_exec];
        g->next_exec = (g->next_exec + 1) % g->nexec;
        HIPCHK(hipGraphLaunch(e, g->stream));
        return 0;
    }
    return run_steps(g, g->stream);
}

int tamd_graph_direct_packets(const tamd_graph* g) { return g && g->half[0] ? pair_direct_packets(g, false) : g && g->direct ? direct_packets(g->direct) : 0; }
int tamd_graph_direct_meta_packets(const tamd_graph* g) { return g && g->half[0] ? pair_direct_packets(g, true) : g && g->direct ? direct_meta_packets(g->direct) : 0; }
const char* tamd_graph_direct_packet_name(const tamd_graph* g, int i) { return g && g->half[0] ? pair_direct_packet_name(g, i) : g && g->direct ? direct_packet_name(g->direct, i) : ""; }

int tamd_graph_direct_timestamps(tamd_graph* g, int passes, double* dur_us, double* gap_us, int max_packets)
{
    if (!g) { set_error("null graph"); return -1; }
    TAMD_ONE_THREAD(g);
    if (bind_device(g)) return -1;
    if (g->half[0]) return pair_direct_timestamps(g, passes, dur_us, gap_us, max_packets);
    if (!g->prepared || !g->direct) { set_error("tamd_graph_direct_timestamps: the graph does not dispatch directly (tamd_options.direct_dispatch)"); return -1; }
    if (!g->inflight.empty()) { set_error("tamd_graph_direct_timestamps while asynchronous runs are in flight"); return -1; }
    if (max_packets < direct_packets(g->direct)) { set_error("tamd_graph_direct_timestamps: %d packets, room for %d", direct_packets(g->direct), max_packets); return -1; }
    if (direct_drain(g)) return -1;
    HIPCHK(hipStreamSynchronize(g->stream));
    g->stream_dirty = false;
    g->out_fresh_in = -1;
    const int n = direct_timestamps(g->direct, passes, dur_us, gap_us);
    if (n < 0) { set_error("direct dispatch: %s", direct_last_error()); return -1; }
    return n;
}
int tamd_graph_slot_timestamps(tamd_graph* g, int passes, double* start_us, double* end_us, int max_stamps)
{
    if (!g) { set_error("null graph"); return -1; }
    TAMD_ONE_THREAD(g);
    if (bind_device(g)) return -1;
    if (!g->prepared || g->half[0]) { set_error("tamd_graph_slot_timestamps: the graph has one launch list (tamd_graph_slots() == 0)"); return -1; }
    if (!g->inflight.empty()) { set_error("tamd_graph_slot_timestamps while asynchronous runs are in flight"); return -1; }
    if (direct_drain(g)) return -1;
    HIPCHK(hipStreamSynchronize(g->stream));
    g->stream_dirty = false;
    g->out_fresh_in = -1;
    return slots_timestamps(g, passes, start_us, end_us, max_stamps);
}
double tamd_graph_prerun_ms(const tamd_graph* g) { return g ? g->prerun_ms : 0.0; }

int tamd_graph_sync(tamd_graph* g)
{
    TAMD_ONE_THREAD(g);
    if (bind_device(g)) return -1;
    if (g->half[0]) return pair_both(g, tamd_graph_sync);
    if (direct_drain(g)) return -1;
    if (g->io[0].direct && !g->inflight.empty() && direct_wait_all(g->io[0].direct)) { set_error("direct dispatch: %s", direct_last_error()); return -1; }
    HIPCHK(hipStreamSynchronize(g->stream));
    g->stream_dirty = false;
    return 0;
}

int tamd_graph_download_outputs(tamd_graph* g)
{
    TAMD_ONE_THREAD(g);
    if (bind_device(g)) return -1;
    if (g->half[0]) return pair_both(g, tamd_graph_download_outputs);
    if (!g->inflight.empty()) { set_error("tamd_graph_download_outputs while asynchronous runs are in flight (they own the pinned buffers): collect them with tamd_graph_wait first"); return -1; }
    if (direct_drain(g)) return -1;
    if (g->out_fresh_in >= 0) {
        for (auto& io : g->outputs)
            if (io.host_out) memcpy(io.host_out, io.pinned[g->out_fresh_in], io.bytes);
        return 0;
    }
    for (auto& io : g->outputs) HIPCHK(hipMemcpyAsync(io.pinned[0], io.stage, io.bytes, hipMemcpyDeviceToHost, g->stream));
    HIPCHK(hipStreamSynchronize(g->stream));
    for (auto& io : g->outputs)
        if (io.host_out) memcpy(io.host_out, io.pinned[0], io.bytes);
    return 0;
}

int tamd_graph_run(tamd_graph* g)
{
    TAMD_ONE_THREAD(g);
    if (!g || !g->prepared) { set_error("graph not prepared"); return -1; }
    if (g->half[0]) return pair_run(g);
    if (!g->inflight.empty()) { set_error("tamd_graph_run while asynchronous runs are in flight: collect them with tamd_graph_wait first"); return -1; }
    if (bind_device(g)) return -1;
    if (direct_drain(g)) return -1;
    static const bool trace = getenv("TAMD_H2H_TRACE") && atoi(getenv("TAMD_H2H_TRACE")) == 1;
    long long t[6] = {0, 0, 0, 0, 0, 0};
    if (trace) t[0] = now_ns();
    for (auto& io : g->inputs) {
        if (!io.host_in) { set_error("input buffer not set"); return -1; }
        memcpy(io.pinned[0], io.host_in, io.bytes);
    }
    if (trace) t[1] = now_ns();
    IoSlot& s = g->io[0];
    if (s.direct) {
        if (drain_stream_if_pending(g)) return -1;
        if (trace) t[2] = now_ns();
        unsigned long long b = 0;
        const int rc = submit_burst(s.direct, &b);
        if (trace) t[3] = now_ns();
        if (rc || direct_wait_burst(s.direct, b)) return direct_abandon(g);
    } else {
        if (trace) t[2] = t[3] = now_ns();
        if (launch_io(g, 0)) return -1;
        HIPCHK(hipStreamSynchronize(g->stream));
    }
    if (trace) t[4] = now_ns();
    g->out_fresh_in = (s.direct && s.zero_copy) ? 0 : -1;
    for (auto& io : g->outputs)
        if (io.host_out) memcpy(io.host_out, io.pinned[0], io.bytes);
    if (trace) {
        t[5] = now_ns();
        for (int i = 0; i < 5; i++) g->h2h_ns[i] += t[i + 1] - t[i];
        g->h2h_runs++;
    }
    return 0;
}

int tamd_graph_run_async(tamd_graph* g)
{
    TAMD_ONE_THREAD(g);
    if (!g || !g->prepared) { set_error("graph not prepared"); return -1; }
    if (bind_device(g)) return -1;
    if (g->half[0]) return pair_run_async(g);
    if (g->inflight.size() >= 2) { set_error("two runs are already in flight: call tamd_graph_wait first"); return -1; }
    if (direct_drain(g)) return -1;
    Inflight f;
    f.io_slot = g->next_io_slot;
    IoSlot& s = g->io[f.io_slot];
    for (auto& io : g->inputs) {
        if (!io.host_in) { set_error("input buffer not set"); return -1; }
        memcpy(io.pinned[f.io_slot], io.host_in, io.bytes);
    }
    for (auto& io : g->outputs) f.host_out.push_back(io.host_out);
    if (g->io[0].direct && g->io[1].direct) {
        if (g->inflight.empty() && drain_stream_if_pending(g)) return -1;
        if (submit_burst(s.direct, &f.burst)) return direct_abandon(g);
        f.direct = true;
    } else {
        if (!s.done) HIPCHK(hipEventCreateWithFlags(&s.done, hipEventDisableTiming));
        g->stream_dirty = true;
        if (launch_io(g, f.io_slot)) return -1;
        f.done = s.done;
        HIPCHK(hipEventRecord(f.done, g->stream));
    }
    g->inflight.push_back(f);
    g->next_io_slot ^= 1;
    return 0;
}

int tamd_graph_wait(tamd_graph* g)
{
    TAMD_ONE_THREAD(g);
    if (g && g->half[0]) return pair_wait(g);
    if (!g || g->inflight.empty()) { set_error("tamd_graph_wait: no run in flight"); return -1; }
    if (bind_device(g)) return -1;
    const Inflight f = g->inflight.front();
    if (f.direct) {
        if (direct_wait_burst(g->io[0].direct, f.burst)) return direct_abandon(g);
    } else
        HIPCHK(hipEventSynchronize(f.done));
    for (size_t i = 0; i < g->outputs.size(); i++)
        if (f.host_out[i]) memcpy(f.host_out[i], g->outputs[i].pinned[f.io_slot], g->outputs[i].bytes);
    g->out_fresh_in = (f.direct && g->io[f.io_slot].zero_copy) ? f.io_slot : -1;
    g->inflight.erase(g->inflight.begin());
    return 0;
}

int tamd_graph_inflight(const tamd_graph* g) { return !g ? 0 : g->half[0] ? tamd_graph_inflight(g->half[0]) : (int)g->inflight.size(); }

int tamd_graph_output_device(tamd_graph* g, int idx, void** dptr, size_t* bytes)
{
    if (!g) { set_error("null graph"); return -1; }
    TAMD_ONE_THREAD(g);
    if (idx < 0 || idx >= (int)g->outputs.size() || !g->prepared) return -1;
    if (g->half[0]) return pair_output_device(g, idx, dptr, bytes);
    if (g->out_fresh_in >= 0 && (bind_device(g) || stage_from_pinned(g))) return -1;
    *dptr = g->outputs[idx].stage;
    *bytes = g->outputs[idx].bytes;
    return 0;
}

void* tamd_graph_stream(tamd_graph* g)
{
    if (g->half[0]) { (void)tamd_graph_stream(g->half[1]); return tamd_graph_stream(g->half[0]); }
    g->stream_exposed = true; g->stream_dirty = true;
    return (void*)g->stream;
}

int tamd_graph_time_launches(tamd_graph* g, int iters, float* total_ms)
{
    TAMD_ONE_THREAD(g);
    if (bind_device(g)) return -1;
    if (g->half[0]) return pair_time_launches(g, iters, total_ms);
    if (g->direct) {
        if (direct_drain(g)) return -1;
        HIPCHK(hipStreamSynchronize(g->stream));
        g->slot_hold = true;
        const auto t0 = std::chrono::steady_clock::now();
        int rc = 0;
        for (int i = 0; i < iters && !rc; i++) rc = tamd_graph_launch(g);
        g->slot_hold = false;
        if (rc || direct_drain(g)) return -1;
        *total_ms = std::chrono::duration<float, std::milli>(std::chrono::steady_clock::now() - t0).count();
        return 0;
    }
    hipEvent_t e0, e1;
    HIPCHK(hipEventCreate(&e0));
    HIPCHK(hipEventCreate(&e1));
    HIPCHK(hipEventRecord(e0, g->stream));
    for (int i = 0; i < iters; i++)
        if (tamd_graph_launch(g)) return -1;
    HIPCHK(hipEventRecord(e1, g->stream));
    HIPCHK(hipEventSynchronize(e1));
    HIPCHK(hipEventElapsedTime(total_ms, e0, e1));
    hipEventDestroy(e0);
    hipEventDestroy(e1);
    return 0;
}

}
```

tengine_amd/csrc/graph_internal.h:

```cpp
#pragma once
#include <mutex>

#include "graph.h"
#include "launch_rec.h"

namespace tamd {

extern std::mutex g_capture_mutex;
const char* last_error();

static inline int esize(int dt) { return (dt == TAMD_DT_FP32 || dt == TAMD_DT_INT32) ? 4 : (dt == TAMD_DT_FP16 ? 2 : 1); }
static inline int cdiv_c(int a, int b) { return a / b; }

int infer_shapes(tamd_graph* g);
int validate_graph(tamd_graph* g);
int plan_i8(tamd_graph* g);
void plan_cache_flush();

int run_steps(tamd_graph* g, hipStream_t s, int io_slot = -1);
int record_pass(tamd_graph* g, int io_slot, std::vector<LaunchRec>* recs);
int direct_selfcheck(tamd_graph* g);
int selfcheck_fill_inputs(tamd_graph* g, unsigned seed, int io_slot = -1);
typedef std::vector<std::vector<unsigned char>> OutputBytes;
int selfcheck_snapshot(const tamd_graph* g, OutputBytes* dst, int io_slot = -1, const std::vector<SlotSpan>* spans = nullptr);
int selfcheck_same(const OutputBytes& want, const OutputBytes& got, const char* fmt);
int build_io_program(tamd_graph* g, int io_slot);
int bind_device(tamd_graph* g);
int direct_drain(tamd_graph* g);
void direct_teardown(tamd_graph* g);
int stage_from_pinned(tamd_graph* g);

void slots_try_build(tamd_graph* g, const std::vector<LaunchRec>& recs, int mode);
void slots_destroy(tamd_graph* g);
int slots_timestamps(tamd_graph* g, int passes, double* start_us, double* end_us, int max_stamps);

int pair_try_prerun(tamd_graph* g, const tamd_options* opt);
int pair_set_input(tamd_graph* g, int idx, const void* host, size_t bytes);
int pair_set_output(tamd_graph* g, int idx, void* host, size_t bytes);
int pair_both(tamd_graph* g, int (*fn)(tamd_graph*));
int pair_run(tamd_graph* g);
int pair_run_async(tamd_graph* g);
int pair_wait(tamd_graph* g);
int pair_direct_packets(const tamd_graph* g, bool meta);
const char* pair_direct_packet_name(const tamd_graph* g, int i);
int pair_direct_timestamps(tamd_graph* g, int passes, double* dur_us, double* gap_us, int max_packets);
int pair_output_device(tamd_graph* g, int idx, void** dptr, size_t* bytes);
int pair_time_launches(tamd_graph* g, int iters, float* total_ms);
int pair_kernel_num(const tamd_graph* g);
int pair_profile(tamd_graph* g, int iters, tamd_kernel_info* out, int max_out);
int pair_read_tensor(tamd_graph* g, int idx, void* host, size_t bytes);
void pair_destroy(tamd_graph* g);

struct OneThread {
    tamd_graph* g;
    bool ok = true, outer = false;
    explicit OneThread(tamd_graph* g_) : g(g_)
    {
        static thread_local char marker;
        const unsigned long me = (unsigned long)(uintptr_t)&marker;
        if (!g) return;
        unsigned long none = 0;
        if (g->owner.compare_exchange_strong(none, me)) outer = true;
        else if (none != me) ok = false;
    }
    ~OneThread() { if (g && outer) g->owner.store(0); }
};

}

#define TAMD_ONE_THREAD(g_)                                                                                                          \
    tamd::OneThread one_thread_(g_);                                                                                                 \
    if (!one_thread_.ok) { tamd::set_error("this tamd_graph is inside a call on another thread: one graph = one thread at a time (include/tengine_amd.h)"); return -1; }
```

tengine_amd/csrc/graph_slots.h:

```cpp
#pragma once
#include <algorithm>
#include <cstddef>
#include <cstdint>
#include <cstring>
#include <vector>

namespace tamd {

struct SlotRange { uintptr_t lo = 0; size_t bytes = 0; };
struct SlotSpan {
    uintptr_t lo = 0, hi = 0;
    size_t off = 0;
    intptr_t delta = 0;
};

template <typename A>
inline SlotRange slot_range_of(const A& a)
{
    SlotRange x;
    x.lo = (uintptr_t)a.base; x.bytes = a.size;
    return x;
}

constexpr size_t kSlotPad = 4096;

inline std::vector<SlotSpan> slot_merge(std::vector<SlotRange> r, size_t* total)
{
    r.erase(std::remove_if(r.begin(), r.end(), [](const SlotRange& x) { return x.bytes == 0 || x.lo == 0; }), r.end());
    std::sort(r.begin(), r.end(), [](const SlotRange& a, const SlotRange& b) { return a.lo < b.lo; });
    std::vector<SlotSpan> spans;
    for (const SlotRange& x : r) {
        if (!spans.empty() && x.lo <= spans.back().hi) spans.back().hi = std::max(spans.back().hi, x.lo + x.bytes);
        else { SlotSpan s; s.lo = x.lo; s.hi = x.lo + x.bytes; spans.push_back(s); }
    }
    size_t at = kSlotPad;
    for (SlotSpan& s : spans) {
        at = ((at + 255) & ~(size_t)255) + (size_t)(s.lo & 255);
        s.off = at;
        at += (size_t)(s.hi - s.lo) + kSlotPad;
    }
    if (total) *total = (at + 255) & ~(size_t)255;
    return spans;
}

inline void slot_place(std::vector<SlotSpan>& spans, uintptr_t block)
{
    for (SlotSpan& s : spans) s.delta = (intptr_t)(block + s.off) - (intptr_t)s.lo;
}

inline const SlotSpan* slot_span_of(const std::vector<SlotSpan>& spans, uintptr_t p)
{
    auto it = std::upper_bound(spans.begin(), spans.end(), p, [](uintptr_t v, const SlotSpan& s) { return v < s.lo; });
    if (it == spans.begin()) return nullptr;
    --it;
    return p < it->hi ? &*it : nullptr;
}

inline uintptr_t slot_moved(const std::vector<SlotSpan>& spans, uintptr_t p)
{
    const SlotSpan* s = slot_span_of(spans, p);
    return s ? (uintptr_t)((intptr_t)p + s->delta) : p;
}

inline int slot_rebase(unsigned char* args, size_t bytes, const std::vector<SlotSpan>& spans)
{
    int moved = 0;
    for (size_t off = 0; off + 8 <= bytes; off += 8) {
        uint64_t v;
        memcpy(&v, args + off, 8);
        const SlotSpan* s = slot_span_of(spans, (uintptr_t)v);
        if (!s) continue;
        v = (uint64_t)((int64_t)v + (int64_t)s->delta);
        memcpy(args + off, &v, 8);
        moved++;
    }
    return moved;
}

inline bool slot_touches(const std::vector<SlotSpan>& spans, uintptr_t lo, size_t bytes)
{
    for (const SlotSpan& s : spans)
        if (lo < s.hi && s.lo < lo + bytes) return true;
    return false;
}

}
```

tengine_amd/csrc/graph_slots.hip:

```cpp
#include "graph.h"
#include "graph_internal.h"
#include "env.h"

#include <stdio.h>
#include <stdlib.h>
#include <string.h>

namespace tamd {

namespace {

void say(const char* why)
{
    if (getenv("TAMD_DEBUG")) fprintf(stderr, "[tamd] slots: the graph stays one launch list: %s\n", why);
}

void add_access(std::vector<SlotRange>& r, const Access& a) { r.push_back(slot_range_of(a)); }

int slots_selfcheck(tamd_graph* g)
{
    OutputBytes want, other, got;
    if (selfcheck_fill_inputs(g, 0x51075A11u) || run_steps(g, g->stream)) return -1;
    HIPCHK(hipStreamSynchronize(g->stream));
    if (selfcheck_snapshot(g, &want)) return -1;
    if (selfcheck_fill_inputs(g, 0x0DDBA11Au) || run_steps(g, g->stream)) return -1;
    HIPCHK(hipStreamSynchronize(g->stream));
    if (selfcheck_snapshot(g, &other)) return -1;
    if (selfcheck_fill_inputs(g, 0x51075A11u)) return -1;
    HIPCHK(hipDeviceSynchronize());
    if (direct_submit(g->direct1) || direct_wait(g->direct1)) { set_error("the pass of slot 1 failed: %s", direct_last_error()); return -1; }
    if (selfcheck_snapshot(g, &got, -1, &g->slot_spans)) return -1;
    if (selfcheck_same(want, got, "slot 1 alone does not reproduce the eager pass (output %zu differs)")) return -1;
    if (selfcheck_snapshot(g, &got)) return -1;
    if (selfcheck_same(other, got, "the pass of slot 1 changed slot 0's output %zu")) return -1;
    for (int k = 0; k < 8; k++)
        if (direct_submit((k & 1) ? g->direct1 : g->direct)) { set_error("the alternating burst failed: %s", direct_last_error()); return -1; }
    if (direct_wait(g->direct) || direct_wait(g->direct1)) { set_error("the alternating burst failed: %s", direct_last_error()); return -1; }
    if (selfcheck_snapshot(g, &got)) return -1;
    if (selfcheck_same(want, got, "a burst of alternating passes leaves other bytes in slot 0 (output %zu differs)")) return -1;
    if (selfcheck_snapshot(g, &got, -1, &g->slot_spans)) return -1;
    if (selfcheck_same(want, got, "a burst of alternating passes leaves other bytes in slot 1 (output %zu differs)")) return -1;
    for (auto& io : g->inputs) HIPCHK(hipMemset(io.stage, 0, io.bytes));
    HIPCHK(hipDeviceSynchronize());
    return 0;
}

}

void slots_try_build(tamd_graph* g, const std::vector<LaunchRec>& recs, int mode)
{
    if (!g->direct || g->is_half || g->inputs.empty() || g->outputs.empty()) { if (!g->direct) say("the list is not dispatched directly"); return; }
    for (auto& t : g->tensors)
        if (t.ttype != TAMD_TT_CONST && t.dtype != TAMD_DT_INT8) { say("not an int8 graph"); return; }
    if (mode != 2) {
        const HTensor& in0 = g->tensors[g->inputs[0].tensor];
        if (in0.dims.empty() || in0.dims[0] != 1) return;
    }
    if (g->had_once) { say("a launch of the plan ran once at prerun (its results exist in one copy)"); return; }
    for (auto& st : g->steps)
        if (step_states_nothing(st)) { say("a launch states nothing of what it reads and writes"); return; }
    std::vector<SlotRange> ranges;
    for (auto* v : {&g->in_steps, &g->steps, &g->out_steps})
        for (auto& st : *v)
            for (auto& w : st.wr) add_access(ranges, w);
    auto is_input_stage = [&](const void* p) {
        for (auto& io : g->inputs)
            if ((const char*)p >= (const char*)io.stage && (const char*)p < (const char*)io.stage + io.bytes) return true;
        return false;
    };
    for (auto& t : g->tensors)
        if (t.ttype != TAMD_TT_CONST && t.dptr && !t.prerun_const && !is_input_stage(t.dptr)) add_access(ranges, access_of(t));
    for (auto& io : g->outputs) {
        SlotRange x;
        x.lo = (uintptr_t)io.stage; x.bytes = io.bytes;
        ranges.push_back(x);
    }
    for (auto& x : ranges)
        for (auto& a : g->arenas)
            if (x.lo >= (uintptr_t)a.base && x.lo < (uintptr_t)a.base + a.used) x.bytes = std::min<size_t>(x.bytes, (uintptr_t)a.base + a.used - x.lo);
    size_t total = 0;
    std::vector<SlotSpan> spans = slot_merge(ranges, &total);
    if (spans.empty()) { say("nothing to re-point"); return; }
    for (auto& io : g->inputs)
        if (slot_touches(spans, (uintptr_t)io.stage, io.bytes)) { say("a launch writes a graph input's staging buffer"); return; }
    for (auto& t : g->tensors)
        if (t.prerun_const && t.dptr && slot_touches(spans, (uintptr_t)t.dptr, 1)) { say("a prerun constant lives in a written buffer"); return; }
    if (hipMalloc(&g->slot_block, total) != hipSuccess) { (void)hipGetLastError(); g->slot_block = nullptr; say("no device memory for the second slot"); return; }
    slot_place(spans, (uintptr_t)g->slot_block);
    bool ok = hipMemset(g->slot_block, 0, total) == hipSuccess;
    for (size_t i = 0; i < spans.size() && ok; i++)
        ok = hipMemcpy((char*)g->slot_block + spans[i].off, (const void*)spans[i].lo, spans[i].hi - spans[i].lo, hipMemcpyDeviceToDevice) == hipSuccess;
    ok = ok && hipDeviceSynchronize() == hipSuccess;
    if (!ok) { (void)hipGetLastError(); say("the copy of the written spans failed"); slots_destroy(g); return; }
    std::vector<LaunchRec> recs1 = recs;
    int moved = 0;
    for (auto& r : recs1) moved += slot_rebase(r.args.data(), r.args.size(), spans);
    if (!moved) { say("no argument points into a written span"); slots_destroy(g); return; }
    const char* why = "";
    g->direct1 = direct_build(g->gpu, g->stream, recs1, &why);
    if (!g->direct1) { say(why); slots_destroy(g); return; }
    g->slot_spans = spans;
    if (slots_selfcheck(g)) {
        fprintf(stderr, "tengine_amd: the second slot is NOT used for this graph: %s (one launch list, as before)\n", last_error());
        slots_destroy(g);
        return;
    }
    if (getenv("TAMD_DEBUG"))
        fprintf(stderr, "[tamd] slots: two passes in flight on two HSA queues; slot 1 owns %zu span(s), %.2f MB, %d argument words re-pointed in %zu launches\n",
                spans.size(), total / 1048576.0, moved, recs1.size());
}

void slots_destroy(tamd_graph* g)
{
    if (g->direct1) { direct_destroy(g->direct1); g->direct1 = nullptr; }
    if (g->slot_block) { (void)hipFree(g->slot_block); g->slot_block = nullptr; }
    g->slot_spans.clear();
    g->slot_turn = 0;
}

int slots_timestamps(tamd_graph* g, int passes, double* start_us, double* end_us, int max_stamps)
{
    if (!g->direct || !g->direct1) { set_error("tamd_graph_slot_timestamps: the graph has one launch list (tamd_graph_slots() == 0)"); return -1; }
    const int n = direct_packets(g->direct);
    if (passes < 1 || (long long)passes * 2 * n > (long long)max_stamps) { set_error("tamd_graph_slot_timestamps: %d rounds of 2 x %d packets, room for %d stamps", passes, n, max_stamps); return -1; }
    const int rc = direct_timestamps_two(g->direct, g->direct1, passes, start_us, end_us);
    if (rc < 0) { set_error("direct dispatch: %s", direct_last_error()); return -1; }
    return rc;
}

}
```

tengine_amd/csrc/launch_rec.h:

```cpp
#pragma once
#include <hip/hip_runtime.h>

#include <cstring>
#include <string>
#include <vector>

namespace tamd {

struct LaunchRec {
    const void* func;
    dim3 grid, block;
    unsigned shmem;
    std::vector<unsigned char> args;
    bool coherent = false;
    bool beside = false;
    bool wrap = false;
};

extern thread_local std::vector<LaunchRec>* g_launch_rec;
extern thread_local bool g_launch_coherent;
inline void launch_rec_coherent() { g_launch_coherent = true; }
extern thread_local bool g_launch_beside;
inline void launch_rec_beside() { g_launch_beside = true; }
inline void launch_rec_clear_flags() { g_launch_coherent = false; g_launch_beside = false; }

template <typename T>
inline void rec_pack(std::vector<unsigned char>& b, const T& v)
{
    const size_t off = (b.size() + alignof(T) - 1) & ~(alignof(T) - 1);
    b.resize(off + sizeof(T));
    memcpy(b.data() + off, &v, sizeof(T));
}

template <typename... P, typename... A>
inline void launch_rec(void (*kernel)(P...), dim3 grid, dim3 block, size_t shmem, hipStream_t s, A&&... a)
{
    static_assert(sizeof...(P) == sizeof...(A), "kernel launched with the wrong number of arguments");
    if (g_launch_rec) {
        LaunchRec r;
        r.func = reinterpret_cast<const void*>(kernel);
        r.grid = grid; r.block = block; r.shmem = (unsigned)shmem;
        (rec_pack<P>(r.args, static_cast<P>(a)), ...);
        r.coherent = g_launch_coherent;
        r.beside = g_launch_beside;
        g_launch_rec->push_back(std::move(r));
    }
    g_launch_coherent = false;
    g_launch_beside = false;
    kernel<<<grid, block, shmem, s>>>(static_cast<P>(a)...);
}

struct DirectProgram;
DirectProgram* direct_build(int gpu, hipStream_t stream, const std::vector<LaunchRec>& recs, const char** why, DirectProgram* share = nullptr);
bool direct_probe(int gpu);
int direct_submit(DirectProgram* p, bool close_burst = false, unsigned long long* burst = nullptr);
int direct_close(DirectProgram* p, unsigned long long* burst);
int direct_wait_burst(DirectProgram* p, unsigned long long burst);
int direct_wait(DirectProgram* p);
int direct_wait_all(DirectProgram* p);
const char* direct_last_error();
int direct_packets(const DirectProgram* p);
const char* direct_packet_name(const DirectProgram* p, int i);
int direct_timestamps(DirectProgram* p, int passes, double* dur_us, double* gap_us);
int direct_timestamps_two(DirectProgram* a, DirectProgram* b, int passes, double* start_us, double* end_us);
int direct_meta_packets(const DirectProgram* p);
void direct_destroy(DirectProgram* p);

}
```

tengine_amd/csrc/plan_cache.hip:

```cpp
#include "graph.h"
#include "graph_internal.h"
#include "env.h"

#include <stdarg.h>
#include <stddef.h>
#include <stdio.h>
#include <string.h>
#include <sys/stat.h>
#include <unistd.h>

#include <algorithm>
#include <cfloat>
#include <chrono>
#include <cmath>
#include <mutex>

#include "epilogue.h"

namespace tamd {

struct PlanCache {
    bool loaded = false, dirty = false;
    std::string path;
    long long stamp = 0;
    std::map<std::string, std::string> kv;
    std::map<std::string, std::string> mine;
};
static std::mutex g_plan_cache_mu;
static long long file_stamp(const std::string& path)
{
    struct stat st;
    if (path.empty() || stat(path.c_str(), &st) != 0) return 0;
    return (long long)st.st_size * 1000003ll ^ (long long)st.st_mtim.tv_sec * 1000000007ll ^ (long long)st.st_mtim.tv_nsec;
}
static std::string plan_cache_header()
{
    return std::string("#tamd-plan v2 gfx950 ") + tamd_version() + " gemm" + std::to_string(conv_igemm_num_cfgs()) + "/" + std::to_string(conv_pgemm_num_variants())
           + " u8" + std::to_string(conv_u8_gemm_num_cfgs()) + "/" + std::to_string(conv_u8_patch_num_cfgs());
}
static void plan_cache_read(const std::string& path, std::map<std::string, std::string>* kv)
{
    FILE* f = path.empty() ? nullptr : fopen(path.c_str(), "r");
    if (!f) return;
    char line[512];
    bool first = true, ok = false;
    while (fgets(line, sizeof(line), f)) {
        std::string l = line;
        while (!l.empty() && (l.back() == '\n' || l.back() == '\r')) l.pop_back();
        if (first) { first = false; ok = l == plan_cache_header(); if (!ok) break; continue; }
        const size_t tab = l.find('\t');
        if (tab == std::string::npos) continue;
        (*kv)[l.substr(0, tab)] = l.substr(tab + 1);
    }
    fclose(f);
    if (!ok) kv->clear();
}
static PlanCache& plan_cache_locked()
{
    static PlanCache pc;
    const char* p = getenv("TAMD_PLAN_CACHE");
    const std::string want = p ? p : "";
    if (!pc.loaded || pc.path != want || (!pc.dirty && file_stamp(want) != pc.stamp)) {
        pc = PlanCache();
        pc.loaded = true; pc.path = want; pc.stamp = file_stamp(want);
        plan_cache_read(want, &pc.kv);
    }
    return pc;
}
static bool plan_cache_get(const std::string& key, std::string* v)
{
    std::lock_guard<std::mutex> lk(g_plan_cache_mu);
    PlanCache& pc = plan_cache_locked();
    auto it = pc.kv.find(key);
    if (pc.path.empty() || it == pc.kv.end()) return false;
    *v = it->second;
    return true;
}
static void plan_cache_put(const std::string& key, const std::string& v)
{
    std::lock_guard<std::mutex> lk(g_plan_cache_mu);
    PlanCache& pc = plan_cache_locked();
    if (pc.path.empty()) return;
    pc.kv[key] = v;
    pc.mine[key] = v;
    pc.dirty = true;
}
void plan_cache_flush()
{
    std::lock_guard<std::mutex> lk(g_plan_cache_mu);
    PlanCache& pc = plan_cache_locked();
    if (pc.path.empty() || !pc.dirty) return;
    std::map<std::string, std::string> merged;
    plan_cache_read(pc.path, &merged);
    for (auto& e : pc.mine) merged[e.first] = e.second;
    const std::string tmp = pc.path + ".tmp." + std::to_string((long)getpid());
    if (FILE* f = fopen(tmp.c_str(), "w")) {
        fprintf(f, "%s\n", plan_cache_header().c_str());
        for (auto& e : merged) fprintf(f, "%s\t%s\n", e.first.c_str(), e.second.c_str());
        fclose(f);
        if (rename(tmp.c_str(), pc.path.c_str()) != 0) (void)remove(tmp.c_str());
    }
    pc.kv = merged;
    pc.dirty = false;
    pc.stamp = file_stamp(pc.path);
}

constexpr size_t kL2FlushBytes = 64u << 20;

static void* l2_flush_buffer()
{
    static std::mutex mu;
    static std::map<int, void*> per_dev;
    int dev = 0;
    if (hipGetDevice(&dev) != hipSuccess) return nullptr;
    std::lock_guard<std::mutex> lk(mu);
    auto it = per_dev.find(dev);
    if (it != per_dev.end()) return it->second;
    void* p = nullptr;
    if (hipMalloc(&p, kL2FlushBytes) != hipSuccess) { (void)hipGetLastError(); p = nullptr; }
    per_dev[dev] = p;
    return p;
}

static bool autotune_cold(tamd_graph* g)
{
    if (g->autotune_cold < 0) {
        const char* e = exp_env("TAMD_AUTOTUNE_COLD");
        size_t bytes = 0;
        for (const HTensor& t : g->tensors)
            bytes += (t.ttype == TAMD_TT_VAR || t.ttype == TAMD_TT_INPUT) && t.n > 0 ? (size_t)t.n * t.h * t.w * (t.cs > 0 ? t.cs : t.c) : t.elems() * (t.dtype == TAMD_DT_FP32 ? 4 : 1);
        g->autotune_cold = e ? (atoi(e) != 0) : bytes > (size_t)(48u << 20);
    }
    return g->autotune_cold == 1;
}

static int time_cold(tamd_graph* g, void* flush, const std::function<hipError_t()>& launch, float* ms_out)
{
    hipEvent_t e0, e1;
    HIPCHK(hipEventCreate(&e0)); HIPCHK(hipEventCreate(&e1));
    const Step* prev = nullptr;
    for (size_t i = g->steps.size(); i-- > 0 && !prev;)
        if (!g->steps[i].once) prev = &g->steps[i];
    float tot = 0.f, worst = 0.f;
    const int reps = 5;
    for (int it = 0; it < reps; it++) {
        float t = 0;
        HIPCHK(hipMemsetAsync(flush, it, kL2FlushBytes, g->stream));
        if (prev) (void)prev->fn(g->stream);
        HIPCHK(hipEventRecord(e0, g->stream));
        (void)launch();
        HIPCHK(hipEventRecord(e1, g->stream));
        HIPCHK(hipEventSynchronize(e1));
        HIPCHK(hipEventElapsedTime(&t, e0, e1));
        tot += t;
        worst = std::max(worst, t);
    }
    hipEventDestroy(e0); hipEventDestroy(e1);
    (void)hipGetLastError();
    *ms_out = (tot - worst) / (reps - 1);
    return 0;
}

static int time_fn(tamd_graph* g, const std::function<hipError_t(hipStream_t)>& fn, float* ms_out)
{
    hipEvent_t e0, e1;
    *ms_out = 1e30f;
    hipError_t err = fn(g->stream);
    if (err == hipSuccess) err = fn(g->stream);
    if (err != hipSuccess) { (void)hipGetLastError(); return 0; }
    HIPCHK(hipEventCreate(&e0)); HIPCHK(hipEventCreate(&e1));
    if (void* flush = autotune_cold(g) ? l2_flush_buffer() : nullptr) {
        hipEventDestroy(e0); hipEventDestroy(e1);
        return time_cold(g, flush, [&]() { return fn(g->stream); }, ms_out);
    }
    float ms = 1e30f;
    int reps = 8;
    for (int round = 0; round < 3; round++) {
        float t = 0;
        HIPCHK(hipEventRecord(e0, g->stream));
        for (int it = 0; it < reps; it++) (void)fn(g->stream);
        HIPCHK(hipEventRecord(e1, g->stream));
        HIPCHK(hipEventSynchronize(e1));
        HIPCHK(hipEventElapsedTime(&t, e0, e1));
        t /= reps;
        if (round == 0 && t <= 0.02f) { reps = 40; continue; }
        ms = std::min(ms, t);
        if (round == 0) round = 1;
    }
    hipEventDestroy(e0); hipEventDestroy(e1);
    *ms_out = ms;
    return 0;
}

bool autotune_enabled()
{
    const char* at_env = getenv("TAMD_AUTOTUNE");
    return !(at_env && atoi(at_env) == 0);
}

int plan_cached(const std::string& key, const std::vector<RaceCand>& cands)
{
    std::string v;
    if (key.empty() || !plan_cache_get(key, &v)) return -1;
    for (size_t c = 0; c < cands.size(); c++)
        if (cands[c].tag == v) return !cands[c].live || cands[c].live() ? (int)c : -1;
    return -1;
}

int plan_race(tamd_graph* g, const std::string& node, const std::vector<RaceCand>& cands, const std::string& key, float margin, bool tune)
{
    if (!tune) return 0;
    const int hit = plan_cached(key, cands);
    if (hit >= 0) return hit;
    int best = 0;
    float best_ms = 1e30f;
    for (size_t c = 0; c < cands.size(); c++) {
        float ms;
        if (time_fn(g, cands[c].fn, &ms)) return -1;
        if (getenv("TAMD_DEBUG"))
            fprintf(stderr, ms > 1e29f ? "[tamd] %s: %s does not launch\n" : "[tamd] %s: %s %.2f us\n", node.c_str(),
                    (cands[c].name.empty() ? cands[c].tag : cands[c].name).c_str(), 1e3 * ms);
        if (ms > 1e29f) continue;
        if (best_ms > 1e29f || ms < best_ms * margin) { best_ms = ms; best = (int)c; }
    }
    if (!key.empty()) plan_cache_put(key, cands[best].tag);
    return best;
}

}
```

Before: 36120 images/s.

## Generalize pass slots to up to four passes in flight with tuned depth

Replaces the single second slot with a vector of pass slots, each with its own rebased buffer block and HSA queue, and rotates submissions across them. Each additional depth is checked against reference outputs and can be timed to choose a depth, which is cached in the plan file. By default the ceiling stays at two unless TAMD_DEEP_SLOTS=1 is set, so deeper overlap is opt-in. Deeper slots cost extra device memory and more prerun selfcheck and timing work.

Result: no change. 36110 images/s, median of 3 (-0.0%).

```diff
diff --git a/include/tengine_amd.h b/include/tengine_amd.h
--- a/include/tengine_amd.h
+++ b/include/tengine_amd.h
@@ -151,6 +151,7 @@
 TAMD_API int tamd_graph_prerun(tamd_graph* g, const tamd_options* opt);
 TAMD_API int tamd_graph_halves(const tamd_graph* g);
 TAMD_API int tamd_graph_slots(const tamd_graph* g);
+TAMD_API int tamd_graph_passes_in_flight(const tamd_graph* g);
 TAMD_API int tamd_graph_input_num(const tamd_graph* g);
 TAMD_API int tamd_graph_output_num(const tamd_graph* g);
 TAMD_API int tamd_graph_input_desc(const tamd_graph* g, int idx, int* dims8, int* dtype);
@@ -169,6 +170,7 @@
 TAMD_API int tamd_graph_direct_timestamps(tamd_graph* g, int passes, double* dur_us, double* gap_us, int max_packets);
 TAMD_API const char* tamd_graph_direct_packet_name(const tamd_graph* g, int i);
 TAMD_API int tamd_graph_slot_timestamps(tamd_graph* g, int passes, double* start_us, double* end_us, int max_stamps);
+TAMD_API int tamd_graph_deep_timestamps(tamd_graph* g, int passes, double* start_us, double* end_us, int max_stamps);
 TAMD_API int tamd_graph_download_outputs(tamd_graph* g);
 TAMD_API int tamd_graph_output_device(tamd_graph* g, int idx, void** dptr, size_t* bytes);
 TAMD_API void* tamd_graph_stream(tamd_graph* g);
diff --git a/tengine_amd/capi.py b/tengine_amd/capi.py
--- a/tengine_amd/capi.py
+++ b/tengine_amd/capi.py
@@ -23,11 +23,11 @@
 EXPORTS = [
     "tamd_device_count", "tamd_init", "tamd_shutdown", "tamd_last_error", "tamd_version", "tamd_op_supported", "tamd_node_supported", "tamd_lut_table", "tamd_interp_table", "tamd_interp_indices", "tamd_shuffle_sources", "tamd_split_table", "tamd_slice_table", "tamd_prelu_slope", "tamd_prelu_table",
     "tamd_graph_create", "tamd_graph_add_tensor", "tamd_graph_add_node", "tamd_graph_set_inputs",
-    "tamd_graph_set_outputs", "tamd_graph_load_tm2", "tamd_graph_set_batch", "tamd_graph_prerun", "tamd_graph_halves", "tamd_graph_slots",
+    "tamd_graph_set_outputs", "tamd_graph_load_tm2", "tamd_graph_set_batch", "tamd_graph_prerun", "tamd_graph_halves", "tamd_graph_slots", "tamd_graph_passes_in_flight",
     "tamd_graph_input_num", "tamd_graph_output_num", "tamd_graph_input_desc", "tamd_graph_output_desc",
     "tamd_graph_set_input", "tamd_graph_set_output", "tamd_graph_run", "tamd_graph_run_async", "tamd_graph_wait", "tamd_graph_inflight", "tamd_graph_upload_inputs",
     "tamd_graph_launch", "tamd_graph_sync", "tamd_graph_direct_packets", "tamd_graph_direct_meta_packets", "tamd_graph_download_outputs", "tamd_graph_output_device",
-    "tamd_graph_direct_timestamps", "tamd_graph_slot_timestamps", "tamd_graph_direct_packet_name", "tamd_graph_stream", "tamd_graph_time_launches", "tamd_graph_prerun_ms", "tamd_graph_kernel_num", "tamd_graph_profile",
+    "tamd_graph_direct_timestamps", "tamd_graph_slot_timestamps", "tamd_graph_deep_timestamps", "tamd_graph_direct_packet_name", "tamd_graph_stream", "tamd_graph_time_launches", "tamd_graph_prerun_ms", "tamd_graph_kernel_num", "tamd_graph_profile",
     "tamd_graph_read_tensor", "tamd_graph_tensor_num", "tamd_graph_tensor_desc", "tamd_graph_destroy",
 ]
 
@@ -62,6 +62,9 @@
         if hasattr(L, "tamd_graph_slots"):
             L.tamd_graph_slot_timestamps.argtypes = [vp, ci, C.POINTER(C.c_double), C.POINTER(C.c_double), ci]
             L.tamd_graph_slots.argtypes = [vp]
+        if hasattr(L, "tamd_graph_passes_in_flight"):
+            L.tamd_graph_deep_timestamps.argtypes = [vp, ci, C.POINTER(C.c_double), C.POINTER(C.c_double), ci]
+            L.tamd_graph_passes_in_flight.argtypes = [vp]
         L.tamd_graph_prerun_ms.restype = C.c_double
         L.tamd_graph_prerun_ms.argtypes = [vp]
         for name, args in {
@@ -199,6 +202,16 @@
     def slots(self):
         return lib().tamd_graph_slots(self._h) if hasattr(lib(), "tamd_graph_slots") else 0
 
+    def passes_in_flight(self):
+        L = lib()
+        return L.tamd_graph_passes_in_flight(self._h) if hasattr(L, "tamd_graph_passes_in_flight") else (2 if self.slots() else 1)
+
+    def deep_timestamps(self, passes=50):
+        n, d = lib().tamd_graph_direct_packets(self._h), self.passes_in_flight()
+        t0, t1 = (C.c_double * (passes * d * n))(), (C.c_double * (passes * d * n))()
+        r = _check(lib().tamd_graph_deep_timestamps(self._h, passes, t0, t1, passes * d * n), "deep_timestamps")
+        return (np.array(t0[:r * d * n]).reshape(r, d, n), np.array(t1[:r * d * n]).reshape(r, d, n))
+
     def slot_timestamps(self, passes=50):
         n = lib().tamd_graph_direct_packets(self._h)
         t0, t1 = (C.c_double * (passes * 2 * n))(), (C.c_double * (passes * 2 * n))()
diff --git a/tengine_amd/csrc/direct.cc b/tengine_amd/csrc/direct.cc
--- a/tengine_amd/csrc/direct.cc
+++ b/tengine_amd/csrc/direct.cc
@@ -345,40 +345,46 @@
     return 0;
 }
 
-int direct_timestamps_two(DirectProgram* a, DirectProgram* b, int passes, double* start_us, double* end_us)
-{
-    const int n = (int)a->pkts.size();
-    if (n == 0 || (int)b->pkts.size() != n || passes < 1 || a->dq == b->dq) { direct_err("two programs of the same list on two queues are needed", 0); return -1; }
-    DirectProgram* prog[2] = {a, b};
-    if (direct_wait_all(a) || direct_wait_all(b)) return -1;
+int direct_timestamps_many(DirectProgram* const* prog, int m, int passes, double* start_us, double* end_us)
+{
+    const int n = m > 0 ? (int)prog[0]->pkts.size() : 0;
+    bool ok = n > 0 && m >= 2 && passes >= 1;
+    for (int k = 0; k < m && ok; k++) {
+        ok = (int)prog[k]->pkts.size() == n;
+        for (int j = 0; j < k && ok; j++) ok = prog[j]->dq != prog[k]->dq;
+    }
+    if (!ok) { direct_err("programs of the same list on queues of their own are needed", m); return -1; }
+    DirectProgram* a = prog[0];
+    auto wait_each = [&](int (*fn)(DirectProgram*)) { for (int k = 0; k < m; k++) if (fn(prog[k])) return -1; return 0; };
+    if (wait_each(direct_wait_all)) return -1;
     uint64_t freq = 0;
     if (hsa_system_get_info(HSA_SYSTEM_INFO_TIMESTAMP_FREQUENCY, &freq) != HSA_STATUS_SUCCESS || !freq) { direct_err("no timestamp frequency", 0); return -1; }
-    for (DirectProgram* p : prog)
-        if (hsa_amd_profiling_set_profiler_enabled(p->dq->q, 1) != HSA_STATUS_SUCCESS) { direct_err("hsa_amd_profiling_set_profiler_enabled", 0); return -1; }
+    for (int k = 0; k < m; k++)
+        if (hsa_amd_profiling_set_profiler_enabled(prog[k]->dq->q, 1) != HSA_STATUS_SUCCESS) { direct_err("hsa_amd_profiling_set_profiler_enabled", 0); return -1; }
     const int extra = 3, all = passes + extra;
-    std::vector<hsa_signal_t> sig((size_t)all * 2 * n);
+    std::vector<hsa_signal_t> sig((size_t)all * m * n);
     for (auto& s : sig)
         if (hsa_signal_create(1, 0, nullptr, &s) != HSA_STATUS_SUCCESS) { direct_err("hsa_signal_create", 0); return -1; }
     int rc = 0;
     for (int ps = 0; ps < all && !rc; ps++) {
-        for (int k = 0; k < 2 && !rc; k++) rc = submit_stamped(prog[k], &sig[((size_t)ps * 2 + k) * n]);
-        if (ps + 1 == extra && !rc) rc = direct_wait(a) || direct_wait(b) ? -1 : 0;
-    }
-    if (!rc) rc = direct_wait(a) || direct_wait(b) ? -1 : 0;
+        for (int k = 0; k < m && !rc; k++) rc = submit_stamped(prog[k], &sig[((size_t)ps * m + k) * n]);
+        if (ps + 1 == extra && !rc) rc = wait_each(direct_wait);
+    }
+    if (!rc) rc = wait_each(direct_wait);
     std::vector<uint64_t> t0(sig.size(), 0), t1(sig.size(), 0);
     for (size_t k = 0; k < sig.size() && !rc; k++) {
         hsa_amd_profiling_dispatch_time_t t{};
         if (hsa_amd_profiling_get_dispatch_time(a->agent, sig[k], &t) != HSA_STATUS_SUCCESS) { direct_err("hsa_amd_profiling_get_dispatch_time", (int)k); rc = -1; break; }
         t0[k] = t.start; t1[k] = t.end;
     }
-    for (DirectProgram* p : prog) (void)hsa_amd_profiling_set_profiler_enabled(p->dq->q, 0);
+    for (int k = 0; k < m; k++) (void)hsa_amd_profiling_set_profiler_enabled(prog[k]->dq->q, 0);
     for (auto& s : sig) (void)hsa_signal_destroy(s);
     if (rc) return -1;
     int first_ok = extra;
     for (size_t k = 0; k < sig.size(); k++)
-        if (t1[k] <= t0[k]) first_ok = std::max(first_ok, (int)(k / ((size_t)2 * n)) + 1);
+        if (t1[k] <= t0[k]) first_ok = std::max(first_ok, (int)(k / ((size_t)m * n)) + 1);
     if (first_ok >= all) { direct_err("no round of the burst carries dispatch stamps throughout", all); return -1; }
-    const size_t first = (size_t)first_ok * 2 * n;
+    const size_t first = (size_t)first_ok * m * n;
     uint64_t origin = ~(uint64_t)0;
     for (size_t k = first; k < sig.size(); k++) origin = std::min(origin, t0[k]);
     for (size_t k = first; k < sig.size(); k++) {
@@ -386,6 +392,12 @@
         end_us[k - first] = 1e6 * (double)(t1[k] - origin) / (double)freq;
     }
     return all - first_ok;
+}
+
+int direct_timestamps_two(DirectProgram* a, DirectProgram* b, int passes, double* start_us, double* end_us)
+{
+    DirectProgram* const prog[2] = {a, b};
+    return direct_timestamps_many(prog, 2, passes, start_us, end_us);
 }
 
 int direct_timestamps(DirectProgram* p, int passes, double* dur_us, double* gap_us)
diff --git a/tengine_amd/csrc/graph.h b/tengine_amd/csrc/graph.h
--- a/tengine_amd/csrc/graph.h
+++ b/tengine_amd/csrc/graph.h
@@ -161,6 +161,13 @@
     int next_exec = 0;
     hipEvent_t done = nullptr;
 };
+
+struct PassSlot {
+    DirectProgram* direct = nullptr;
+    void* block = nullptr;
+    std::vector<SlotSpan> spans;
+};
+constexpr int kMaxPassSlots = 4;
 
 struct Inflight {
     int io_slot = 0;
@@ -209,9 +216,7 @@
     int next_io_slot = 0;
     std::vector<tamd::Inflight> inflight;
     tamd::DirectProgram* direct = nullptr;
-    tamd::DirectProgram* direct1 = nullptr;
-    void* slot_block = nullptr;
-    std::vector<tamd::SlotSpan> slot_spans;
+    std::vector<tamd::PassSlot> pass_slots;
     int slot_turn = 0;
     bool slot_hold = false;
     bool had_once = false;
diff --git a/tengine_amd/csrc/graph.hip b/tengine_amd/csrc/graph.hip
--- a/tengine_amd/csrc/graph.hip
+++ b/tengine_amd/csrc/graph.hip
@@ -418,7 +418,8 @@
 }
 
 int tamd_graph_halves(const tamd_graph* g) { return g && g->half[0] ? 2 : 0; }
-int tamd_graph_slots(const tamd_graph* g) { return g && !g->half[0] && g->direct && g->direct1 ? 2 : 0; }
+int tamd_graph_slots(const tamd_graph* g) { return tamd_graph_passes_in_flight(g) > 1 ? 2 : 0; }
+int tamd_graph_passes_in_flight(const tamd_graph* g) { return g && !g->half[0] && g->direct ? 1 + (int)g->pass_slots.size() : 1; }
 int tamd_graph_input_num(const tamd_graph* g) { return (int)g->inputs.size(); }
 int tamd_graph_output_num(const tamd_graph* g) { return (int)g->outputs.size(); }
 
diff --git a/tengine_amd/csrc/graph_exec.hip b/tengine_amd/csrc/graph_exec.hip
--- a/tengine_amd/csrc/graph_exec.hip
+++ b/tengine_amd/csrc/graph_exec.hip
@@ -223,7 +223,9 @@
 int direct_drain(tamd_graph* g)
 {
     if (g->direct && g->direct_busy) {
-        if (direct_wait(g->direct) || (g->direct1 && direct_wait(g->direct1))) { set_error("direct dispatch: %s", direct_last_error()); return -1; }
+        bool bad = direct_wait(g->direct) != 0;
+        for (auto& s : g->pass_slots) bad = bad || direct_wait(s.direct);
+        if (bad) { set_error("direct dispatch: %s", direct_last_error()); return -1; }
         g->direct_busy = false;
     }
     g->slot_turn = 0;
@@ -312,7 +314,10 @@
         if (!g->direct_busy) { HIPCHK(hipStreamSynchronize(g->stream)); g->stream_dirty = false; }
         g->direct_busy = true;
         DirectProgram* p = g->direct;
-        if (g->direct1 && !g->slot_hold) { if (g->slot_turn) p = g->direct1; g->slot_turn ^= 1; }
+        if (!g->pass_slots.empty() && !g->slot_hold) {
+            if (g->slot_turn) p = g->pass_slots[g->slot_turn - 1].direct;
+            g->slot_turn = (g->slot_turn + 1) % (1 + (int)g->pass_slots.size());
+        }
         if (direct_submit(p)) { set_error("direct dispatch: %s", direct_last_error()); return -1; }
         return 0;
     }
@@ -358,7 +363,20 @@
     HIPCHK(hipStreamSynchronize(g->stream));
     g->stream_dirty = false;
     g->out_fresh_in = -1;
-    return slots_timestamps(g, passes, start_us, end_us, max_stamps);
+    return slots_timestamps(g, 2, passes, start_us, end_us, max_stamps, "tamd_graph_slot_timestamps");
+}
+int tamd_graph_deep_timestamps(tamd_graph* g, int passes, double* start_us, double* end_us, int max_stamps)
+{
+    if (!g) { set_error("null graph"); return -1; }
+    TAMD_ONE_THREAD(g);
+    if (bind_device(g)) return -1;
+    if (!g->prepared || g->half[0]) { set_error("tamd_graph_deep_timestamps: the graph has one launch list (tamd_graph_slots() == 0)"); return -1; }
+    if (!g->inflight.empty()) { set_error("tamd_graph_deep_timestamps while asynchronous runs are in flight"); return -1; }
+    if (direct_drain(g)) return -1;
+    HIPCHK(hipStreamSynchronize(g->stream));
+    g->stream_dirty = false;
+    g->out_fresh_in = -1;
+    return slots_timestamps(g, kMaxPassSlots, passes, start_us, end_us, max_stamps, "tamd_graph_deep_timestamps");
 }
 double tamd_graph_prerun_ms(const tamd_graph* g) { return g ? g->prerun_ms : 0.0; }
 
diff --git a/tengine_amd/csrc/graph_internal.h b/tengine_amd/csrc/graph_internal.h
--- a/tengine_amd/csrc/graph_internal.h
+++ b/tengine_amd/csrc/graph_internal.h
@@ -16,6 +16,8 @@
 int validate_graph(tamd_graph* g);
 int plan_i8(tamd_graph* g);
 void plan_cache_flush();
+bool plan_cache_get(const std::string& key, std::string* v);
+void plan_cache_put(const std::string& key, const std::string& v);
 
 int run_steps(tamd_graph* g, hipStream_t s, int io_slot = -1);
 int record_pass(tamd_graph* g, int io_slot, std::vector<LaunchRec>* recs);
@@ -32,7 +34,7 @@
 
 void slots_try_build(tamd_graph* g, const std::vector<LaunchRec>& recs, int mode);
 void slots_destroy(tamd_graph* g);
-int slots_timestamps(tamd_graph* g, int passes, double* start_us, double* end_us, int max_stamps);
+int slots_timestamps(tamd_graph* g, int depth, int passes, double* start_us, double* end_us, int max_stamps, const char* who);
 
 int pair_try_prerun(tamd_graph* g, const tamd_options* opt);
 int pair_set_input(tamd_graph* g, int idx, const void* host, size_t bytes);
diff --git a/tengine_amd/csrc/graph_slots.h b/tengine_amd/csrc/graph_slots.h
--- a/tengine_amd/csrc/graph_slots.h
+++ b/tengine_amd/csrc/graph_slots.h
@@ -48,6 +48,12 @@
     for (SlotSpan& s : spans) s.delta = (intptr_t)(block + s.off) - (intptr_t)s.lo;
 }
 
+inline std::vector<SlotSpan> slot_placed(std::vector<SlotSpan> spans, uintptr_t block)
+{
+    slot_place(spans, block);
+    return spans;
+}
+
 inline const SlotSpan* slot_span_of(const std::vector<SlotSpan>& spans, uintptr_t p)
 {
     auto it = std::upper_bound(spans.begin(), spans.end(), p, [](uintptr_t v, const SlotSpan& s) { return v < s.lo; });
@@ -77,6 +83,14 @@
     return moved;
 }
 
+inline std::vector<unsigned char> slot_rebased(const std::vector<unsigned char>& original, const std::vector<SlotSpan>& spans, int* moved)
+{
+    std::vector<unsigned char> args = original;
+    const int n = slot_rebase(args.data(), args.size(), spans);
+    if (moved) *moved += n;
+    return args;
+}
+
 inline bool slot_touches(const std::vector<SlotSpan>& spans, uintptr_t lo, size_t bytes)
 {
     for (const SlotSpan& s : spans)
diff --git a/tengine_amd/csrc/graph_slots.hip b/tengine_amd/csrc/graph_slots.hip
--- a/tengine_amd/csrc/graph_slots.hip
+++ b/tengine_amd/csrc/graph_slots.hip
@@ -6,6 +6,8 @@
 #include <stdlib.h>
 #include <string.h>
 
+#include <chrono>
+
 namespace tamd {
 
 namespace {
@@ -17,32 +19,128 @@
 
 void add_access(std::vector<SlotRange>& r, const Access& a) { r.push_back(slot_range_of(a)); }
 
-int slots_selfcheck(tamd_graph* g)
-{
-    OutputBytes want, other, got;
-    if (selfcheck_fill_inputs(g, 0x51075A11u) || run_steps(g, g->stream)) return -1;
-    HIPCHK(hipStreamSynchronize(g->stream));
-    if (selfcheck_snapshot(g, &want)) return -1;
-    if (selfcheck_fill_inputs(g, 0x0DDBA11Au) || run_steps(g, g->stream)) return -1;
-    HIPCHK(hipStreamSynchronize(g->stream));
-    if (selfcheck_snapshot(g, &other)) return -1;
+DirectProgram* slot_program(tamd_graph* g, int k) { return k == 0 ? g->direct : g->pass_slots[k - 1].direct; }
+
+int rotating_burst(tamd_graph* g, int d, int passes)
+{
+    for (int k = 0; k < passes; k++)
+        if (direct_submit(slot_program(g, k % d))) { set_error("the rotating burst failed: %s", direct_last_error()); return -1; }
+    for (int k = 0; k < d; k++)
+        if (direct_wait(slot_program(g, k))) { set_error("the rotating burst failed: %s", direct_last_error()); return -1; }
+    return 0;
+}
+
+int every_slot_holds(tamd_graph* g, int d, int except, const OutputBytes& want, const char* fmt)
+{
+    OutputBytes got;
+    for (int k = 0; k < d; k++) {
+        if (k == except) continue;
+        if (selfcheck_snapshot(g, &got, -1, k ? &g->pass_slots[k - 1].spans : nullptr)) return -1;
+        for (size_t i = 0; i < want.size(); i++)
+            if (want[i] != got[i]) { set_error(fmt, i, k); return -1; }
+    }
+    return 0;
+}
+
+int slot_selfcheck(tamd_graph* g, int d, const OutputBytes& want, const OutputBytes& other)
+{
+    OutputBytes got;
+    if (selfcheck_fill_inputs(g, 0x0DDBA11Au)) return -1;
+    HIPCHK(hipDeviceSynchronize());
+    if (rotating_burst(g, d - 1, d - 1)) return -1;
+    if (every_slot_holds(g, d - 1, -1, other, "a proven slot does not hold the second input's result (output %zu, slot %d)")) return -1;
     if (selfcheck_fill_inputs(g, 0x51075A11u)) return -1;
     HIPCHK(hipDeviceSynchronize());
-    if (direct_submit(g->direct1) || direct_wait(g->direct1)) { set_error("the pass of slot 1 failed: %s", direct_last_error()); return -1; }
-    if (selfcheck_snapshot(g, &got, -1, &g->slot_spans)) return -1;
-    if (selfcheck_same(want, got, "slot 1 alone does not reproduce the eager pass (output %zu differs)")) return -1;
-    if (selfcheck_snapshot(g, &got)) return -1;
-    if (selfcheck_same(other, got, "the pass of slot 1 changed slot 0's output %zu")) return -1;
-    for (int k = 0; k < 8; k++)
-        if (direct_submit((k & 1) ? g->direct1 : g->direct)) { set_error("the alternating burst failed: %s", direct_last_error()); return -1; }
-    if (direct_wait(g->direct) || direct_wait(g->direct1)) { set_error("the alternating burst failed: %s", direct_last_error()); return -1; }
-    if (selfcheck_snapshot(g, &got)) return -1;
-    if (selfcheck_same(want, got, "a burst of alternating passes leaves other bytes in slot 0 (output %zu differs)")) return -1;
-    if (selfcheck_snapshot(g, &got, -1, &g->slot_spans)) return -1;
-    if (selfcheck_same(want, got, "a burst of alternating passes leaves other bytes in slot 1 (output %zu differs)")) return -1;
-    for (auto& io : g->inputs) HIPCHK(hipMemset(io.stage, 0, io.bytes));
-    HIPCHK(hipDeviceSynchronize());
-    return 0;
+    DirectProgram* p = slot_program(g, d - 1);
+    if (direct_submit(p) || direct_wait(p)) { set_error("the pass of slot %d failed: %s", d - 1, direct_last_error()); return -1; }
+    if (selfcheck_snapshot(g, &got, -1, &g->pass_slots[d - 2].spans)) return -1;
+    if (selfcheck_same(want, got, "the new slot alone does not reproduce the eager pass (output %zu differs)")) return -1;
+    if (every_slot_holds(g, d, d - 1, other, "the pass of the new slot changed output %zu of slot %d")) return -1;
+    if (rotating_burst(g, d, 2 * d + 1)) return -1;
+    if (every_slot_holds(g, d, -1, want, "a burst of rotating passes leaves other bytes in output %zu of slot %d")) return -1;
+    return 0;
+}
+
+void slot_release(PassSlot& s)
+{
+    if (s.direct) { direct_destroy(s.direct); s.direct = nullptr; }
+    if (s.block) { (void)hipFree(s.block); s.block = nullptr; }
+    s.spans.clear();
+}
+
+bool slot_build(tamd_graph* g, const std::vector<LaunchRec>& recs, const std::vector<SlotSpan>& merged, size_t total, PassSlot* s, int* moved)
+{
+    if (hipMalloc(&s->block, total) != hipSuccess) { (void)hipGetLastError(); s->block = nullptr; say("no device memory for one more slot"); return false; }
+    s->spans = slot_placed(merged, (uintptr_t)s->block);
+    bool ok = hipMemset(s->block, 0, total) == hipSuccess;
+    for (size_t i = 0; i < s->spans.size() && ok; i++)
+        ok = hipMemcpy((char*)s->block + s->spans[i].off, (const void*)s->spans[i].lo, s->spans[i].hi - s->spans[i].lo, hipMemcpyDeviceToDevice) == hipSuccess;
+    ok = ok && hipDeviceSynchronize() == hipSuccess;
+    if (!ok) { (void)hipGetLastError(); say("the copy of the written spans failed"); slot_release(*s); return false; }
+    std::vector<LaunchRec> mine = recs;
+    *moved = 0;
+    for (size_t i = 0; i < recs.size(); i++) mine[i].args = slot_rebased(recs[i].args, s->spans, moved);
+    if (!*moved) { say("no argument points into a written span"); slot_release(*s); return false; }
+    const char* why = "";
+    s->direct = direct_build(g->gpu, g->stream, mine, &why);
+    if (!s->direct) { say(why); slot_release(*s); return false; }
+    return true;
+}
+
+std::string list_identity(const tamd_graph* g, const std::vector<LaunchRec>& recs)
+{
+    uint64_t h = 1469598103934665603ull;
+    auto mix = [&](const void* p, size_t n) { for (size_t i = 0; i < n; i++) { h ^= ((const unsigned char*)p)[i]; h *= 1099511628211ull; } };
+    for (size_t i = 0; i < recs.size(); i++) {
+        const char* name = direct_packet_name(g->direct, (int)i);
+        mix(name, strlen(name));
+        const unsigned v[8] = {recs[i].grid.x, recs[i].grid.y, recs[i].grid.z, recs[i].block.x, recs[i].block.y, recs[i].block.z, recs[i].shmem, (unsigned)recs[i].args.size()};
+        mix(v, sizeof(v));
+    }
+    char key[96];
+    snprintf(key, sizeof(key), "slots|%zu launches|%016llx", recs.size(), (unsigned long long)h);
+    return key;
+}
+
+constexpr int kRacePasses = 200;
+constexpr double kDepthMargin = 0.06;
+
+int burst_us(tamd_graph* g, int d, double* us_per_pass)
+{
+    double best = 1e30;
+    if (rotating_burst(g, d, 4 * d)) return -1;
+    for (int rep = 0; rep < 3; rep++) {
+        const auto t0 = std::chrono::steady_clock::now();
+        if (rotating_burst(g, d, kRacePasses)) return -1;
+        best = std::min(best, std::chrono::duration<double, std::micro>(std::chrono::steady_clock::now() - t0).count() / kRacePasses);
+    }
+    *us_per_pass = best;
+    return 0;
+}
+
+int cached_depth(const std::string& key)
+{
+    std::string v;
+    if (!autotune_enabled() || !plan_cache_get(key, &v)) return 0;
+    const int d = atoi(v.c_str());
+    return d >= 2 && d <= kMaxPassSlots ? d : 0;
+}
+
+int slots_choose_depth(tamd_graph* g, const std::string& key, int proven)
+{
+    if (proven <= 2 || !autotune_enabled()) return std::min(proven, 2);
+    int depth = 2;
+    double t_depth = 0;
+    if (burst_us(g, 2, &t_depth)) return 2;
+    for (int d = 3; d <= proven; d++) {
+        double t = 0;
+        if (burst_us(g, d, &t)) return depth;
+        if (getenv("TAMD_DEBUG")) fprintf(stderr, "[tamd] slots: depth %d %.2f us per pass, depth %d %.2f\n", depth, t_depth, d, t);
+        if (!(t < t_depth * (1.0 - kDepthMargin))) break;
+        depth = d; t_depth = t;
+    }
+    plan_cache_put(key, std::to_string(depth));
+    return depth;
 }
 
 }
@@ -56,6 +154,14 @@
         const HTensor& in0 = g->tensors[g->inputs[0].tensor];
         if (in0.dims.empty() || in0.dims[0] != 1) return;
     }
+    const char* pin = tamd_pin("pass_slots");
+    const int pinned = pin ? std::max(1, std::min(kMaxPassSlots, atoi(pin))) : 0;
+    if (pinned == 1) { say("pinned to one pass at a time (TAMD_PIN=pass_slots=1)"); return; }
+    const std::string key = pinned ? std::string() : list_identity(g, recs);
+    const int cached = pinned ? 0 : cached_depth(key);
+    const char* deep = getenv("TAMD_DEEP_SLOTS");
+    const int ceiling = deep && atoi(deep) == 1 && autotune_enabled() ? kMaxPassSlots : 2;
+    const int want_depth = pinned ? pinned : std::min(ceiling, cached ? cached : kMaxPassSlots);
     if (g->had_once) { say("a launch of the plan ran once at prerun (its results exist in one copy)"); return; }
     for (auto& st : g->steps)
         if (step_states_nothing(st)) { say("a launch states nothing of what it reads and writes"); return; }
@@ -79,51 +185,64 @@
         for (auto& a : g->arenas)
             if (x.lo >= (uintptr_t)a.base && x.lo < (uintptr_t)a.base + a.used) x.bytes = std::min<size_t>(x.bytes, (uintptr_t)a.base + a.used - x.lo);
     size_t total = 0;
-    std::vector<SlotSpan> spans = slot_merge(ranges, &total);
+    const std::vector<SlotSpan> spans = slot_merge(ranges, &total);
     if (spans.empty()) { say("nothing to re-point"); return; }
     for (auto& io : g->inputs)
         if (slot_touches(spans, (uintptr_t)io.stage, io.bytes)) { say("a launch writes a graph input's staging buffer"); return; }
     for (auto& t : g->tensors)
         if (t.prerun_const && t.dptr && slot_touches(spans, (uintptr_t)t.dptr, 1)) { say("a prerun constant lives in a written buffer"); return; }
-    if (hipMalloc(&g->slot_block, total) != hipSuccess) { (void)hipGetLastError(); g->slot_block = nullptr; say("no device memory for the second slot"); return; }
-    slot_place(spans, (uintptr_t)g->slot_block);
-    bool ok = hipMemset(g->slot_block, 0, total) == hipSuccess;
-    for (size_t i = 0; i < spans.size() && ok; i++)
-        ok = hipMemcpy((char*)g->slot_block + spans[i].off, (const void*)spans[i].lo, spans[i].hi - spans[i].lo, hipMemcpyDeviceToDevice) == hipSuccess;
-    ok = ok && hipDeviceSynchronize() == hipSuccess;
-    if (!ok) { (void)hipGetLastError(); say("the copy of the written spans failed"); slots_destroy(g); return; }
-    std::vector<LaunchRec> recs1 = recs;
+    OutputBytes want, other;
+    auto eager = [&](unsigned seed, OutputBytes* out) {
+        if (selfcheck_fill_inputs(g, seed) || run_steps(g, g->stream)) return -1;
+        HIPCHK(hipStreamSynchronize(g->stream));
+        return selfcheck_snapshot(g, out);
+    };
+    if (eager(0x51075A11u, &want) || eager(0x0DDBA11Au, &other)) { say(last_error()); return; }
     int moved = 0;
-    for (auto& r : recs1) moved += slot_rebase(r.args.data(), r.args.size(), spans);
-    if (!moved) { say("no argument points into a written span"); slots_destroy(g); return; }
-    const char* why = "";
-    g->direct1 = direct_build(g->gpu, g->stream, recs1, &why);
-    if (!g->direct1) { say(why); slots_destroy(g); return; }
-    g->slot_spans = spans;
-    if (slots_selfcheck(g)) {
-        fprintf(stderr, "tengine_amd: the second slot is NOT used for this graph: %s (one launch list, as before)\n", last_error());
-        slots_destroy(g);
-        return;
+    g->pass_slots.reserve(kMaxPassSlots - 1);
+    for (int d = 2; d <= want_depth; d++) {
+        PassSlot s;
+        if (!slot_build(g, recs, spans, total, &s, &moved)) break;
+        g->pass_slots.push_back(s);
+        if (slot_selfcheck(g, d, want, other)) {
+            if (d == 2) fprintf(stderr, "tengine_amd: the second slot is NOT used for this graph: %s (one launch list, as before)\n", last_error());
+            else if (getenv("TAMD_DEBUG")) fprintf(stderr, "[tamd] slots: slot %d is not used: %s (the graph keeps %d passes in flight)\n", d - 1, last_error(), d - 1);
+            slot_release(g->pass_slots.back());
+            g->pass_slots.pop_back();
+            break;
+        }
+    }
+    for (auto& io : g->inputs) (void)hipMemset(io.stage, 0, io.bytes);
+    (void)hipDeviceSynchronize();
+    (void)hipGetLastError();
+    const int proven = 1 + (int)g->pass_slots.size();
+    if (proven < 2) return;
+    const int depth = pinned || proven == cached ? proven : slots_choose_depth(g, key, proven);
+    while ((int)g->pass_slots.size() > depth - 1) {
+        slot_release(g->pass_slots.back());
+        g->pass_slots.pop_back();
     }
     if (getenv("TAMD_DEBUG"))
-        fprintf(stderr, "[tamd] slots: two passes in flight on two HSA queues; slot 1 owns %zu span(s), %.2f MB, %d argument words re-pointed in %zu launches\n",
-                spans.size(), total / 1048576.0, moved, recs1.size());
+        fprintf(stderr, "[tamd] slots: %d passes in flight on %d HSA queues (%d proved themselves%s%s); every extra slot owns %zu span(s), %.2f MB, %d argument words re-pointed in %zu launches\n",
+                depth, depth, proven, pinned ? ", depth pinned" : "", cached ? ", depth from the plan file" : "", spans.size(), total / 1048576.0, moved, recs.size());
 }
 
 void slots_destroy(tamd_graph* g)
 {
-    if (g->direct1) { direct_destroy(g->direct1); g->direct1 = nullptr; }
-    if (g->slot_block) { (void)hipFree(g->slot_block); g->slot_block = nullptr; }
-    g->slot_spans.clear();
+    for (size_t k = g->pass_slots.size(); k-- > 0;) slot_release(g->pass_slots[k]);
+    g->pass_slots.clear();
     g->slot_turn = 0;
 }
 
-int slots_timestamps(tamd_graph* g, int passes, double* start_us, double* end_us, int max_stamps)
-{
-    if (!g->direct || !g->direct1) { set_error("tamd_graph_slot_timestamps: the graph has one launch list (tamd_graph_slots() == 0)"); return -1; }
+int slots_timestamps(tamd_graph* g, int depth, int passes, double* start_us, double* end_us, int max_stamps, const char* who)
+{
+    if (!g->direct || g->pass_slots.empty()) { set_error("%s: the graph has one launch list (tamd_graph_slots() == 0)", who); return -1; }
+    depth = std::min(depth, 1 + (int)g->pass_slots.size());
     const int n = direct_packets(g->direct);
-    if (passes < 1 || (long long)passes * 2 * n > (long long)max_stamps) { set_error("tamd_graph_slot_timestamps: %d rounds of 2 x %d packets, room for %d stamps", passes, n, max_stamps); return -1; }
-    const int rc = direct_timestamps_two(g->direct, g->direct1, passes, start_us, end_us);
+    if (passes < 1 || (long long)passes * depth * n > (long long)max_stamps) { set_error("%s: %d rounds of %d x %d packets, room for %d stamps", who, passes, depth, n, max_stamps); return -1; }
+    std::vector<DirectProgram*> progs;
+    for (int k = 0; k < depth; k++) progs.push_back(slot_program(g, k));
+    const int rc = direct_timestamps_many(progs.data(), depth, passes, start_us, end_us);
     if (rc < 0) { set_error("direct dispatch: %s", direct_last_error()); return -1; }
     return rc;
 }
diff --git a/tengine_amd/csrc/launch_rec.h b/tengine_amd/csrc/launch_rec.h
--- a/tengine_amd/csrc/launch_rec.h
+++ b/tengine_amd/csrc/launch_rec.h
@@ -63,6 +63,7 @@
 const char* direct_packet_name(const DirectProgram* p, int i);
 int direct_timestamps(DirectProgram* p, int passes, double* dur_us, double* gap_us);
 int direct_timestamps_two(DirectProgram* a, DirectProgram* b, int passes, double* start_us, double* end_us);
+int direct_timestamps_many(DirectProgram* const* prog, int m, int passes, double* start_us, double* end_us);
 int direct_meta_packets(const DirectProgram* p);
 void direct_destroy(DirectProgram* p);
 
diff --git a/tengine_amd/csrc/plan_cache.hip b/tengine_amd/csrc/plan_cache.hip
--- a/tengine_amd/csrc/plan_cache.hip
+++ b/tengine_amd/csrc/plan_cache.hip
@@ -67,7 +67,7 @@
     }
     return pc;
 }
-static bool plan_cache_get(const std::string& key, std::string* v)
+bool plan_cache_get(const std::string& key, std::string* v)
 {
     std::lock_guard<std::mutex> lk(g_plan_cache_mu);
     PlanCache& pc = plan_cache_locked();
@@ -76,7 +76,7 @@
     *v = it->second;
     return true;
 }
-static void plan_cache_put(const std::string& key, const std::string& v)
+void plan_cache_put(const std::string& key, const std::string& v)
 {
     std::lock_guard<std::mutex> lk(g_plan_cache_mu);
     PlanCache& pc = plan_cache_locked();
```
